# 10XGenomics/scan-rs

Measured on NVIDIA B200. Metric: normalize+PCA cells/s, 1.3Mx33.5k, k=10, higher is better.
Workload: dtype f64

## Files before the change

### profiles/microbench/ring_rate.cu

```cuda
#include <cstdio>
#include <cstdint>
#include <cuda_runtime.h>
#include "../../scan_rs_b200/csrc/tc05.cuh"
using namespace tc05;

template <int NSTG, int MPS, int PW, bool SPIN_PROD>
__global__ void __launch_bounds__(32 * (2 + NSTG * PW), 1) k_ring(int stages, long long *out) {
    extern __shared__ __align__(1024) unsigned char smem[];
    __shared__ unsigned long long full[NSTG], empty[NSTG], done;
    __shared__ uint32_t tslot;
    const uint32_t tid = threadIdx.x, warp = tid >> 5, lane = tid & 31;
    for (uint32_t i = tid; i < 96 * 1024 / 4; i += blockDim.x) reinterpret_cast<uint32_t *>(smem)[i] = 0x01010101u;
    if (tid == 0) {
        for (int i = 0; i < NSTG; i++) { mbar_init(smem_u32(&full[i]), PW); mbar_init(smem_u32(&empty[i]), 1); }
        mbar_init(smem_u32(&done), 1);
        mbar_init_fence();
    }
    if (warp == 0) tmem_alloc_512(smem_u32(&tslot));
    fence_async_smem();
    fence_before_sync();
    __syncthreads();
    fence_after_sync();
    const uint32_t tmem = tslot;
    const uint32_t full0 = smem_u32(full), empty0 = smem_u32(empty);
    if (warp == 1) {
        const uint32_t idesc = instr_desc_i8(128, 144, false, false);
        const uint32_t a16 = smem_u32(smem) >> 4, b16 = a16 + (65536 >> 4);
        const uint64_t da_hi = smem_desc(0, 2048, 128), db_hi = smem_desc(0, 144 / 8 * 128, 128);
        const long long t0 = clock64();
        for (int s = 0; s < stages; s++) {
            const uint32_t ss = s % NSTG;
            mbar_spin(full0 + 8 * ss, (s / NSTG) & 1u);
            fence_after_sync();
            if (elect_one()) {
#pragma unroll
                for (int t = 0; t < MPS; t++) mma_i8(tmem, da_hi | (a16 + ss * 256 + (t & 3) * 64), db_hi | (b16 + (t & 7) * 288), idesc, 1u);
                commit(empty0 + 8 * ss);
            }
            __syncwarp();
        }
        if (elect_one()) commit(smem_u32(&done));
        __syncwarp();
        mbar_wait(smem_u32(&done), 0);
        if (lane == 0 && blockIdx.x == 0) out[0] = clock64() - t0;
    } else if (warp >= 2) {
        const int p = warp - 2, ss = p / PW;
        int fills = 0;
        for (int s = ss; s < stages; s += NSTG, fills++) {
            if (fills > 0) { if (SPIN_PROD) mbar_spin(empty0 + 8 * ss, (fills - 1) & 1u); else mbar_wait(empty0 + 8 * ss, (fills - 1) & 1u); }
            fence_async_smem();
            __syncwarp();
            if (lane == 0) mbar_arrive(full0 + 8 * ss);
        }
    }
    __syncthreads();
    if (warp == 0) tmem_dealloc_512(tmem);
}

template <int NSTG, int MPS, int PW, bool SPIN>
void run(long long *d) {
    const int stages = 4096;
    auto k = k_ring<NSTG, MPS, PW, SPIN>;
    cudaFuncSetAttribute(k, cudaFuncAttributeMaxDynamicSharedMemorySize, 96 * 1024);
    k<<<148, 32 * (2 + NSTG * PW), 96 * 1024>>>(stages, d);
    cudaError_t e = cudaDeviceSynchronize();
    long long h = 0;
    cudaMemcpy(&h, d, 8, cudaMemcpyDeviceToHost);
    printf("stages in ring %2d, MMAs per stage %2d, producer warps per stage %d, producers %s: %6.1f cycles per MMA (floor 72.1)  %s\n", NSTG, MPS, PW,
           SPIN ? "spin    " : "try_wait", (double)h / stages / MPS, cudaGetErrorString(e));
}

int main() {
    long long *d;
    cudaMalloc(&d, 8);
    run<4, 4, 2, false>(d);
    run<4, 4, 2, true>(d);
    run<4, 4, 1, false>(d);
    run<8, 2, 1, false>(d);
    run<8, 4, 1, false>(d);
    run<8, 4, 2, false>(d);
    run<4, 8, 2, false>(d);
    run<2, 8, 4, false>(d);
    run<3, 12, 4, false>(d);
    run<3, 12, 4, true>(d);
    run<2, 16, 4, false>(d);
    return 0;
}
```

### scan_rs_b200/csrc/common.cuh

```cuda
#pragma once
#include <cuda_runtime.h>
#include <cublas_v2.h>
#include <cusolverDn.h>
#include "nccl_shim.h"

#include <cstdarg>
#include <cstdint>
#include <cstdio>
#include <cstring>
#include <memory>
#include <algorithm>
#include <string>
#include <vector>

#include "../../include/scanb200.h"
#include "gather_units.h"

typedef uint32_t u32;
typedef uint64_t u64;

void sb_set_error(const char *fmt, ...);
int sb_fail(int code, const char *fmt, ...);

#define SB_CUDA(expr)                                                                         \
    do {                                                                                      \
        cudaError_t _e = (expr);                                                              \
        if (_e != cudaSuccess)                                                                \
            return sb_fail(_e == cudaErrorMemoryAllocation ? SB_ERR_OOM : SB_ERR_CUDA,        \
                           "CUDA error %s at %s:%d: %s", cudaGetErrorName(_e), __FILE__,      \
                           __LINE__, cudaGetErrorString(_e));                                 \
    } while (0)
#define SB_CUBLAS(expr)                                                                       \
    do {                                                                                      \
        cublasStatus_t _s = (expr);                                                           \
        if (_s != CUBLAS_STATUS_SUCCESS)                                                      \
            return sb_fail(SB_ERR_LINALG, "cuBLAS error %d at %s:%d", (int)_s, __FILE__, __LINE__); \
    } while (0)
#define SB_CUSOLVER(expr)                                                                     \
    do {                                                                                      \
        cusolverStatus_t _s = (expr);                                                         \
        if (_s != CUSOLVER_STATUS_SUCCESS)                                                    \
            return sb_fail(SB_ERR_LINALG, "cuSOLVER error %d at %s:%d", (int)_s, __FILE__, __LINE__); \
    } while (0)
#define SB_NCCL(expr)                                                                         \
    do {                                                                                      \
        ncclResult_t _r = (expr);                                                             \
        if (_r != ncclSuccess)                                                                \
            return sb_fail(SB_ERR_NCCL, "NCCL error %s at %s:%d", ncclGetErrorString(_r),     \
                           __FILE__, __LINE__);                                               \
    } while (0)
#define SB_TRY(expr)                 \
    do {                             \
        int _rc = (expr);            \
        if (_rc != SB_OK) return _rc; \
    } while (0)

cudaStream_t sb_alloc_stream();
cudaMemPool_t sb_alloc_pool();
void sb_set_alloc_stream(cudaStream_t s, cudaMemPool_t pool = nullptr);
bool sb_stream_alive(cudaStream_t s);
void *sb_cache_take(cudaStream_t st, size_t bytes);
bool sb_cache_give(cudaStream_t st, void *p, size_t bytes);
void sb_cache_flush(cudaStream_t st);
void sb_cache_configure(cudaStream_t st, size_t cap_bytes);
#define SB_CACHE_MIN_BYTES ((size_t)1 << 20)
void sb_stream_register(cudaStream_t s, bool alive);

template <typename T>
struct DevBuf {
    T *p = nullptr;
    size_t n = 0;
    cudaStream_t st = nullptr;
    DevBuf() {}
    DevBuf(const DevBuf &) = delete;
    DevBuf &operator=(const DevBuf &) = delete;
    ~DevBuf() { release(); }
    void release() {
        if (p && sb_stream_alive(st)) {
            const size_t bytes = (n ? n : 1) * sizeof(T);
            if (bytes < SB_CACHE_MIN_BYTES || !sb_cache_give(st, p, bytes)) cudaFreeAsync(p, st);
        }
        p = nullptr;
        n = 0;
    }
    int alloc(size_t count) {
        release();
        n = count;
        if (count == 0) count = 1;
        st = sb_alloc_stream();
        if (count * sizeof(T) >= SB_CACHE_MIN_BYTES) {
            p = static_cast<T *>(sb_cache_take(st, count * sizeof(T)));
            if (p) return SB_OK;
        }
        cudaMemPool_t pool = sb_alloc_pool();
        cudaError_t e = pool ? cudaMallocFromPoolAsync((void **)&p, count * sizeof(T), pool, st) : cudaMallocAsync((void **)&p, count * sizeof(T), st);
        if (e == cudaErrorMemoryAllocation) {
            cudaGetLastError();
            sb_cache_flush(st);
            e = pool ? cudaMallocFromPoolAsync((void **)&p, count * sizeof(T), pool, st) : cudaMallocAsync((void **)&p, count * sizeof(T), st);
        }
        if (e != cudaSuccess) {
            p = nullptr;
            n = 0;
            cudaGetLastError();
            return sb_fail(e == cudaErrorMemoryAllocation ? SB_ERR_OOM : SB_ERR_CUDA,
                           "cudaMallocAsync of %zu bytes failed: %s", count * sizeof(T), cudaGetErrorString(e));
        }
        return SB_OK;
    }
    int ensure(size_t count) { return count <= n && p ? SB_OK : alloc(count); }
    void swap(DevBuf &o) {
        T *tp = p; p = o.p; o.p = tp;
        size_t tn = n; n = o.n; o.n = tn;
        cudaStream_t ts = st; st = o.st; o.st = ts;
    }
};

enum Phase { PH_SPMM_T = 0, PH_SPMM_N, PH_MOMENTS, PH_REDUCE, PH_DENSE, PH_COMM, PH_UPLOAD, PH_BUILD, PH_OUTPUT, PH_COUNT };

struct sb_ctx {
    int device = 0;
    int sm_count = 148;
    size_t l2_bytes = 0;
    cudaStream_t stream = nullptr;
    cudaMemPool_t pool = nullptr;
    cudaStream_t copy_stream = nullptr;
    cudaStream_t aux_stream = nullptr;
    cudaEvent_t ev_fork = nullptr, ev_join = nullptr;
    bool overlap = false;
    bool overlap_t = false;
    cublasHandle_t cublas = nullptr;
    cusolverDnHandle_t cusolver = nullptr;
    ncclComm_t comm = nullptr;
    int nranks = 1, rank = 0;
    int dense_cap = 2048;
    double dense_min_density = 0.12;
    bool panel_i8 = false;
    int dense_max_count = 15;
    int panel_mode = 2;
    int pl_debug = 0;
    int pl_variant = 3;
    int plane_items_per_cta = 48;
    int plane_cap = 12288;
    int plane_levels = 6;
    double plane_min_density = 0.01;
    bool gemm_skinny = true;
    bool eig_host = true;
    void *eig_pinned = nullptr;
    size_t eig_pinned_bytes = 0;
    int eig_host_declined = 0;
    int upload_chunks = 8;
    bool upload_sync = true;
    bool gather_defer = true;
    int gather_calibrate = 1;
    double gather_seg_cost = 0.0;
    double gather_flush_cost = 5.0;
    int gather_items_per_cta = 1;
    bool use_gather = true;
    bool direct_projection = false;
    bool verify_projection = false;
    bool eig_jacobi = false;
    bool own_dense = true;
    double last_cond_r = 0.0, last_probe_resid = 0.0;
    int last_fallbacks = 0;
    bool profile_on = false;
    std::vector<std::pair<int, std::pair<cudaEvent_t, cudaEvent_t>>> pending;
    std::vector<cudaEvent_t> event_pool;
    sb_profile prof;
    cudaEvent_t t0 = nullptr, t1 = nullptr;
    DevBuf<char> flush_buf;
    DevBuf<char> scratch;
    DevBuf<double> syrk_parts;
    void *pinned = nullptr;
    std::vector<double> omega_cache;
    u64 omega_seed = ~0ull, omega_rows = 0, omega_cols = 0;
    DevBuf<double> omega_dev;
    u64 omega_dev_seed = ~0ull, omega_dev_rows = 0, omega_dev_cols = 0;
};

#define SB_GENE_BITS 22
#define SB_GENE_MASK 0x3FFFFFu
#define SB_MAX_PANEL_CELLS 1024
#define GA_TBLOCK 16384

#define PL_MAX_LEVELS 6
struct PlUnitT {
    u32 g0, nlev;
    u32 lev[3], nkb[3];
    u32 cta0, nctas;
};
struct PlUnitN {
    u32 g0, nlev;
    u32 mt[PL_MAX_LEVELS];
    u32 cta0, nctas;
};
struct PlItem {
    u32 unit, t0, t1;
};
struct PlaneSet {
    bool active = false;
    u32 L = 0;
    u32 G[PL_MAX_LEVELS] = {0, 0, 0, 0, 0, 0};
    u64 ntiles = 0;
    DevBuf<u32> bits[PL_MAX_LEVELS];
    DevBuf<char> units_t, units_n, items_t, items_n;
    DevBuf<u32> counter;
    mutable DevBuf<signed char> ws_bd, ws_bn;
    mutable DevBuf<double> ws_part, ws_scale2;
    mutable DevBuf<unsigned long long> ws_colmax;
    mutable DevBuf<int> ws_ex;
    u32 n_units_t = 0, n_units_n = 0, n_items_t = 0, n_items_n = 0, t_grid = 0, n_grid = 0;
};

struct GatherLayout {
    bool ready = false;
    u32 rows = 0;
    u32 npanels = 0;
    u64 nnz = 0;
    const uint2 *ent = nullptr;
    DevBuf<uint2> ent_own;
    DevBuf<GUnit> units;
    u32 n_units = 0;
    u32 grid = 0;
    DevBuf<u32> cta_first;
    u32 n_items = 0;
    mutable DevBuf<u32> tickets;
    mutable u32 ticket_base = 0;
    DevBuf<u32> slot_gene;
};

struct sb_mat {
    sb_ctx *ctx = nullptr;
    u32 m = 0;
    u64 n = 0;
    u64 n_global = 0;
    u64 cell_offset = 0;
    u64 nnz = 0;
    DevBuf<u64> cm_ptr;
    DevBuf<uint2> cm;
    u32 pc = 0, np = 0, ur = 1;
    DevBuf<uint2> gm;
    DevBuf<u64> gm_base;
    DevBuf<u64> unit_ptr;
    bool have_full_gm = false;
    u32 gd = 0;
    u32 dense_max_count = 15;
    DevBuf<unsigned char> D;
    DevBuf<u32> hot_idx;
    DevBuf<u32> hot_of_gene;
    PlaneSet pl;
    u64 cold_nnz = 0;
    DevBuf<u64> cold_cm_ptr;
    DevBuf<uint2> cold_cm;
    DevBuf<uint2> cold_gm;
    DevBuf<u64> cold_gm_base;
    GatherLayout gn, gt;
    DevBuf<u32> slot_of_gene;
    std::vector<u64> t_seg_len, t_seg_runs;
    std::vector<GUnit> t_units_host;
    std::vector<u32> t_first_host;
    std::vector<double> t_rate;
    int t_calibrated = 0;
    DevBuf<u32> cell_tot;
    bool have_cell_tot = false;
};
#define SB_DENSE_MAX_COUNT 15u
#define SB_DENSE_LUT 16

struct sb_nmat {
    sb_mat *mat = nullptr;
    sb_ctx *ctx = nullptr;
    int kind = 1;
    int log_base = 0;
    DevBuf<double> col_scale;
    DevBuf<double> l1c, inv_l1c;
    DevBuf<double> lk;
    DevBuf<double> row_scale;
    bool has_row_scale = false;
    bool has_offset = false;
    bool v_ones = true;
    DevBuf<double> u;
    DevBuf<double> v;
};

void prof_begin(sb_ctx *ctx, int phase);
void prof_end(sb_ctx *ctx, int phase);
void prof_collect(sb_ctx *ctx);
static inline void count_launch(sb_ctx *ctx, bool own = true) {
    ctx->prof.kernel_launches++;
    if (own) ctx->prof.own_kernel_launches++;
}
struct ProfScope {
    sb_ctx *c;
    int ph;
    ProfScope(sb_ctx *ctx, int phase) : c(ctx), ph(phase) { prof_begin(c, ph); }
    ~ProfScope() { prof_end(c, ph); }
};

int ctx_scratch(sb_ctx *ctx, size_t bytes, void **out);
int comm_allreduce_f64(sb_ctx *ctx, double *buf, size_t count);
int comm_allreduce_u64(sb_ctx *ctx, u64 *buf, size_t count);
int comm_allreduce_max_i32(sb_ctx *ctx, int *host_val);
int comm_allgather_u64_host(sb_ctx *ctx, u64 mine, std::vector<u64> &all);
int agree_status(sb_ctx *ctx, int rc, const char *what);
double percentile_of(std::vector<double> &v, double q);

#define SB_ENTER(ctx_ptr)                         \
    do {                                          \
        SB_CUDA(cudaSetDevice((ctx_ptr)->device)); \
        sb_set_alloc_stream((ctx_ptr)->stream, (ctx_ptr)->pool); \
    } while (0)

struct TraceScope {
    sb_ctx *c;
    const char *name;
    double t0;
    static bool on();
    static int level();
    static double now();
    TraceScope(sb_ctx *ctx, const char *n) : c(ctx), name(n), t0(0) {
        if (on()) {
            cudaStreamSynchronize(c->stream);
            t0 = now();
        }
    }
    ~TraceScope() {
        if (on()) {
            cudaStreamSynchronize(c->stream);
            fprintf(stderr, "[scanb200] %-28s %8.2f ms\n", name, (now() - t0) * 1e3);
        }
    }
};

struct SyncScope {
    sb_ctx *c;
    const char *name;
    double t0;
    SyncScope(sb_ctx *ctx, const char *n) : c(ctx), name(n), t0(0) {
        cudaStreamSynchronize(c->stream);
        if (TraceScope::on()) t0 = TraceScope::now();
    }
    ~SyncScope() {
        cudaStreamSynchronize(c->stream);
        if (TraceScope::on()) fprintf(stderr, "[scanb200] %-28s %8.2f ms\n", name, (TraceScope::now() - t0) * 1e3);
    }
};

static inline unsigned cdiv(u64 a, u64 b) { return (unsigned)((a + b - 1) / b); }
```

### scan_rs_b200/csrc/planes.cu

```cuda
#include <numeric>

#include "common.cuh"
#include "map.cuh"
#include "tc05.cuh"

using namespace tc05;

#define PL_TILE 128u
#define PL_COLS 20u
#define PL_DIG 7u
#define PL_NCOL 144u
#define PL_FIX 54
#define PL_NONE 0xFFFFFFFFu

#define PT_RANGE 1024u
#define PT_B_BYTES (PT_RANGE * PL_NCOL)
#define PT_KCHUNK_BYTES (PL_NCOL / 8 * 128)
#define PT_WORDS 2u
#define PT_STAGE_BYTES (PL_TILE * 32u * PT_WORDS)
#define PT_NSTAGES 8u
#define PT_SUB 2u
#define PT_NSTG (PT_NSTAGES / PT_SUB)
#define PT_PROD_WARPS PT_NSTAGES
#define PL_EPI_WARPS 4u
#define PL_PROD_WARPS 8u
#define PL_THREADS ((PL_EPI_WARPS + 1 + PL_PROD_WARPS) * 32)

#define PN_GROUP 384u
#define PN_A_BYTES (3u * 4096u)
#define PN_B_BYTES (32u * PL_NCOL)
#define PN_STAGE_BYTES (PN_A_BYTES + PN_B_BYTES)
#define PN_NSTAGES 12u
#define PN_SUB 4u
#define PN_NSTG (PN_NSTAGES / PN_SUB)
#define PN_CELLGRP_BYTES (PL_NCOL / 16 * 128)

struct PlDev {
    u32 *bits[PL_MAX_LEVELS];
    u32 G[PL_MAX_LEVELS];
    u32 L;
    u64 ntiles;
    u64 n;
};

static PlDev make_pldev(const sb_mat *mt) {
    PlDev d;
    memset(&d, 0, sizeof(d));
    d.L = mt->pl.L;
    d.ntiles = mt->pl.ntiles;
    d.n = mt->n;
    for (u32 k = 0; k < mt->pl.L; k++) {
        d.bits[k] = mt->pl.bits[k].p;
        d.G[k] = mt->pl.G[k];
    }
    return d;
}

__global__ void k_pl_level_hist(const u64 *__restrict__ ptr, const uint2 *__restrict__ cm, u64 n, u32 m, u32 L, unsigned long long *__restrict__ hist) {
    u64 warp = ((u64)blockIdx.x * blockDim.x + threadIdx.x) >> 5;
    u64 nwarps = ((u64)gridDim.x * blockDim.x) >> 5;
    int lane = threadIdx.x & 31;
    for (u64 c = warp; c < n; c += nwarps) {
        const u64 s = ptr[c], e = ptr[c + 1];
        for (u64 k = s + lane; k < e; k += 32) {
            const uint2 z = cm[k];
            if (z.y >= 1 && z.y <= L) atomicAdd(&hist[(size_t)(z.y - 1) * m + z.x], 1ull);
        }
    }
}

static void units_round(std::vector<u32> &nctas, const std::vector<double> &cost, u32 total) {
    const size_t U = cost.size();
    nctas.assign(U, 1);
    if (U == 0) return;
    double sum = 0.0;
    for (double c : cost) sum += c;
    if (U >= total || sum <= 0.0) return;
    std::vector<double> ideal(U);
    u32 used = 0;
    for (size_t i = 0; i < U; i++) {
        ideal[i] = cost[i] / sum * total;
        nctas[i] = std::max<u32>(1, (u32)ideal[i]);
        used += nctas[i];
    }
    while (used > total) {
        size_t best = 0;
        double worst = -1e300;
        for (size_t i = 0; i < U; i++)
            if (nctas[i] > 1 && (double)nctas[i] - ideal[i] > worst) { worst = (double)nctas[i] - ideal[i]; best = i; }
        nctas[best]--;
        used--;
    }
    while (used < total) {
        size_t best = 0;
        double worst = -1e300;
        for (size_t i = 0; i < U; i++)
            if (ideal[i] - (double)nctas[i] > worst) { worst = ideal[i] - (double)nctas[i]; best = i; }
        nctas[best]++;
        used++;
    }
}

int planes_select(sb_mat *mt, u64 c0, u64 c1) {
    sb_ctx *ctx = mt->ctx;
    PlaneSet &pl = mt->pl;
    pl.active = false;
    pl.L = 0;
    const u32 m = mt->m;
    const u32 Lmax = (u32)std::min<int>(std::max(ctx->plane_levels, 1), PL_MAX_LEVELS);
    if (m < 128 || mt->n_global == 0 || ctx->plane_cap < 128) return SB_OK;
    SyncScope tr(ctx, "build: plane selection");
    DevBuf<u64> d_hist;
    const size_t hn = (size_t)Lmax * m + 1;
    SB_TRY(d_hist.alloc(hn));
    SB_CUDA(cudaMemsetAsync(d_hist.p, 0, hn * sizeof(u64), ctx->stream));
    if (c1 > c0) {
        ProfScope ps(ctx, PH_REDUCE);
        u64 blocks = std::min<u64>(((c1 - c0) * 32 + 255) / 256, (u64)ctx->sm_count * 16);
        k_pl_level_hist<<<(unsigned)std::max<u64>(1, blocks), 256, 0, ctx->stream>>>(mt->cm_ptr.p + c0, mt->cm.p, c1 - c0, m, Lmax,
                                                                                     (unsigned long long *)d_hist.p);
        count_launch(ctx);
    }
    const u64 sample = c1 - c0;
    SB_CUDA(cudaMemcpyAsync(d_hist.p + (hn - 1), &sample, sizeof(u64), cudaMemcpyHostToDevice, ctx->stream));
    SB_TRY(comm_allreduce_u64(ctx, d_hist.p, hn));
    std::vector<u64> h(hn);
    SB_CUDA(cudaMemcpyAsync(h.data(), d_hist.p, hn * sizeof(u64), cudaMemcpyDeviceToHost, ctx->stream));
    SB_CUDA(cudaStreamSynchronize(ctx->stream));
    const double cells = (double)h[hn - 1];
    if (cells <= 0.0) return SB_OK;
    std::vector<u64> tot(m, 0);
    for (u32 k = 0; k < Lmax; k++)
        for (u32 g = 0; g < m; g++) tot[g] += h[(size_t)k * m + g];
    std::vector<u32> order(m);
    std::iota(order.begin(), order.end(), 0u);
    std::stable_sort(order.begin(), order.end(), [&](u32 a, u32 b) { return tot[a] > tot[b]; });
    const u32 cap = std::min<u32>((u32)ctx->plane_cap, m) & ~127u;
    const double thr = ctx->plane_min_density * cells;
    u32 prev = cap;
    u32 L = 0;
    for (u32 k = 0; k < Lmax; k++) {
        u32 G = 0;
        for (u32 b0 = 0; b0 + 128 <= prev; b0 += 128) {
            double s = 0.0;
            for (u32 r = b0; r < b0 + 128; r++) s += (double)h[(size_t)k * m + order[r]];
            if (s / 128.0 < thr) break;
            G = b0 + 128;
        }
        if (G == 0) break;
        pl.G[k] = G;
        prev = G;
        L = k + 1;
    }
    if (L == 0) return SB_OK;
    pl.L = L;
    pl.ntiles = (mt->n + PL_TILE - 1) / PL_TILE;
    const u32 G1 = pl.G[0];
    std::vector<u32> hot(order.begin(), order.begin() + G1), hot_of(m, PL_NONE);
    for (u32 r = 0; r < G1; r++) hot_of[hot[r]] = r;
    SB_TRY(mt->hot_idx.alloc(G1));
    SB_TRY(mt->hot_of_gene.alloc(m));
    SB_CUDA(cudaMemcpyAsync(mt->hot_idx.p, hot.data(), G1 * sizeof(u32), cudaMemcpyHostToDevice, ctx->stream));
    SB_CUDA(cudaMemcpyAsync(mt->hot_of_gene.p, hot_of.data(), (size_t)m * sizeof(u32), cudaMemcpyHostToDevice, ctx->stream));
    for (u32 k = 0; k < L; k++) {
        const size_t words = std::max<size_t>(1, (size_t)pl.ntiles * (pl.G[k] / 32) * PL_TILE);
        SB_TRY(pl.bits[k].alloc(words));
        SB_CUDA(cudaMemsetAsync(pl.bits[k].p, 0, words * sizeof(u32), ctx->stream));
    }
    std::vector<PlUnitT> ut;
    std::vector<double> cost;
    for (u32 g0 = 0; g0 < G1; g0 += PT_RANGE) {
        std::vector<u32> lv;
        for (u32 k = 0; k < L; k++)
            if (pl.G[k] > g0) lv.push_back(k);
        for (size_t i = 0; i < lv.size(); i += 3) {
            PlUnitT u;
            memset(&u, 0, sizeof(u));
            u.g0 = g0;
            double c = 0.0;
            for (size_t j = i; j < std::min(lv.size(), i + 3); j++) {
                const u32 genes = std::min(pl.G[lv[j]], g0 + PT_RANGE) - g0;
                u.lev[u.nlev] = lv[j];
                u.nkb[u.nlev] = genes / 32;
                u.nlev++;
                c += genes;
            }
            c += (u.nlev > 1 ? 250.0 : 100.0) * u.nlev;
            ut.push_back(u);
            cost.push_back(c);
        }
    }
    {
        double total = 0.0;
        for (double c : cost) total += c * (double)pl.ntiles;
        const double target = std::max(1.0, total / ((double)ctx->sm_count * (double)std::max(1, ctx->plane_items_per_cta)));
        std::vector<u32> uo(ut.size());
        std::iota(uo.begin(), uo.end(), 0u);
        std::stable_sort(uo.begin(), uo.end(), [&](u32 x, u32 y) { return cost[x] > cost[y]; });
        std::vector<PlItem> items;
        for (u32 ui : uo) {
            const u64 per = std::max<u64>(1, (u64)(target / cost[ui] + 0.5));
            for (u64 t0 = 0; t0 < pl.ntiles; t0 += per) {
                PlItem it;
                it.unit = ui;
                it.t0 = (u32)t0;
                it.t1 = (u32)std::min<u64>(pl.ntiles, t0 + per);
                items.push_back(it);
            }
        }
        pl.n_units_t = (u32)ut.size();
        SB_TRY(pl.units_t.alloc(std::max<size_t>(1, ut.size()) * sizeof(PlUnitT)));
        if (!ut.empty()) SB_CUDA(cudaMemcpyAsync(pl.units_t.p, ut.data(), ut.size() * sizeof(PlUnitT), cudaMemcpyHostToDevice, ctx->stream));
        pl.n_items_t = (u32)items.size();
        pl.t_grid = (u32)std::min<size_t>((size_t)ctx->sm_count, std::max<size_t>(1, items.size()));
        SB_TRY(pl.items_t.alloc(std::max<size_t>(1, items.size()) * sizeof(PlItem)));
        if (!items.empty()) SB_CUDA(cudaMemcpyAsync(pl.items_t.p, items.data(), items.size() * sizeof(PlItem), cudaMemcpyHostToDevice, ctx->stream));
        SB_TRY(pl.counter.alloc(4));
        SB_CUDA(cudaStreamSynchronize(ctx->stream));
    }
    std::vector<u32> nc;
    u32 at = 0;
    std::vector<PlUnitN> un;
    cost.clear();
    for (u32 g0 = 0; g0 < G1; g0 += PN_GROUP) {
        PlUnitN u;
        memset(&u, 0, sizeof(u));
        u.g0 = g0;
        double c = 0.0;
        for (u32 k = 0; k < L && pl.G[k] > g0; k++) {
            u.mt[k] = (std::min(pl.G[k], g0 + PN_GROUP) - g0) / 128;
            u.nlev = k + 1;
            c += u.mt[k] + 0.5;
        }
        un.push_back(u);
        cost.push_back(c);
    }
    {
        double total = 0.0;
        for (double c : cost) total += c * (double)pl.ntiles;
        const double target = std::max(1.0, total / ((double)ctx->sm_count * 10.0));
        std::vector<u32> uo(un.size());
        std::iota(uo.begin(), uo.end(), 0u);
        std::stable_sort(uo.begin(), uo.end(), [&](u32 x, u32 y) { return cost[x] > cost[y]; });
        std::vector<PlItem> items;
        for (u32 ui : uo) {
            const u64 per = std::min<u64>(std::max<u64>(1, (u64)(target / cost[ui] + 0.5)), (1u << 24) / PL_TILE);
            for (u64 t0 = 0; t0 < pl.ntiles; t0 += per) {
                PlItem it;
                it.unit = ui;
                it.t0 = (u32)t0;
                it.t1 = (u32)std::min<u64>(pl.ntiles, t0 + per);
                items.push_back(it);
            }
        }
        pl.n_items_n = (u32)items.size();
        pl.n_grid = (u32)std::min<size_t>((size_t)ctx->sm_count, std::max<size_t>(1, items.size()));
        SB_TRY(pl.items_n.alloc(std::max<size_t>(1, items.size()) * sizeof(PlItem)));
        if (!items.empty()) SB_CUDA(cudaMemcpyAsync(pl.items_n.p, items.data(), items.size() * sizeof(PlItem), cudaMemcpyHostToDevice, ctx->stream));
        SB_CUDA(cudaStreamSynchronize(ctx->stream));
    }
    pl.n_units_n = (u32)un.size();
    SB_TRY(pl.units_n.alloc(std::max<size_t>(1, un.size()) * sizeof(PlUnitN)));
    SB_CUDA(cudaMemcpyAsync(pl.units_n.p, un.data(), un.size() * sizeof(PlUnitN), cudaMemcpyHostToDevice, ctx->stream));
    SB_CUDA(cudaStreamSynchronize(ctx->stream));
    pl.active = true;
    mt->gd = G1;
    if (TraceScope::on()) {
        fprintf(stderr, "[scanb200] planes: L=%u G =", L);
        for (u32 k = 0; k < L; k++) fprintf(stderr, " %u", pl.G[k]);
        fprintf(stderr, "  (T units %u / %u CTAs, N units %u / %u CTAs)\n", pl.n_units_t, pl.t_grid, pl.n_units_n, pl.n_grid);
    }
    return SB_OK;
}

__global__ void k_split_planes(const u64 *__restrict__ ptr, const uint2 *__restrict__ cm, u64 n, u64 cbase, const u32 *__restrict__ rank_of_gene,
                               PlDev pl, const u64 *__restrict__ new_ptr, u32 *__restrict__ counts, uint2 *__restrict__ out) {
    u64 warp = ((u64)blockIdx.x * blockDim.x + threadIdx.x) >> 5;
    u64 nwarps = ((u64)gridDim.x * blockDim.x) >> 5;
    int lane = threadIdx.x & 31;
    for (u64 c = warp; c < n; c += nwarps) {
        const u64 s = ptr[c], e = ptr[c + 1];
        const u64 wpos = new_ptr ? new_ptr[c] : 0;
        const u64 cell = cbase + c, tile = cell / PL_TILE;
        const u32 cl = (u32)(cell % PL_TILE);
        u32 total = 0;
        for (u64 k0 = s; k0 < e; k0 += 32) {
            const u64 k = k0 + lane;
            const bool valid = k < e;
            const uint2 z = valid ? cm[k] : make_uint2(0, 0);
            const u32 r = valid ? rank_of_gene[z.x] : PL_NONE;
            const bool dense = valid && r != PL_NONE && z.y >= 1 && z.y <= pl.L && r < pl.G[z.y - 1];
            const bool cold = valid && !dense;
            if (out && dense) {
                const u32 lv = z.y - 1;
                atomicOr(pl.bits[lv] + ((tile * (pl.G[lv] / 32) + (r >> 5)) * PL_TILE + cl), 1u << (r & 31));
            }
            const unsigned mask = __ballot_sync(0xffffffffu, cold);
            if (out && cold) out[wpos + total + __popc(mask & ((1u << lane) - 1u))] = z;
            total += __popc(mask);
        }
        if (counts && lane == 0) counts[c] = total;
    }
}

int planes_split_launch(sb_mat *mt, u64 c0, u64 nc, const u64 *new_ptr, u32 *counts, uint2 *out) {
    sb_ctx *ctx = mt->ctx;
    if (nc == 0) return SB_OK;
    if (c0 % PL_TILE) return sb_fail(SB_ERR_UNSUPPORTED, "planes_split: range start %llu is not a multiple of 128", (unsigned long long)c0);
    u64 blocks = std::min<u64>((nc * 32 + 255) / 256, (u64)ctx->sm_count * 16);
    k_split_planes<<<(unsigned)std::max<u64>(1, blocks), 256, 0, ctx->stream>>>(mt->cm_ptr.p + c0, mt->cm.p, nc, c0, mt->hot_of_gene.p, make_pldev(mt),
                                                                                new_ptr, counts, out);
    count_launch(ctx);
    SB_CUDA(cudaGetLastError());
    return SB_OK;
}

__device__ __forceinline__ double finite_or_zero(double x) { return (x == x && fabs(x) < 1.0e300) ? x : 0.0; }

__device__ __forceinline__ void digits7(long long q, signed char (&d)[PL_DIG]) {
#pragma unroll
    for (u32 s = 0; s < PL_DIG; s++) {
        const long long t = ((q + 128) & 255) - 128;
        d[s] = (signed char)t;
        q = (q - t) >> 8;
    }
}

__device__ __forceinline__ void atomic_max_abs(unsigned long long *slot, double v) {
    atomicMax(slot, (unsigned long long)__double_as_longlong(fabs(v)));
}

__global__ void k_pl_scales(const unsigned long long *__restrict__ colmax_bits, double *__restrict__ scale2, int *__restrict__ ex) {
    const u32 c = threadIdx.x;
    if (c >= PL_COLS) return;
    const double mx = __longlong_as_double((long long)colmax_bits[c]);
    int e = 0;
    if (mx > 0.0) frexp(mx, &e);
    scale2[c] = ldexp(1.0, e - PL_FIX);
    ex[c] = PL_FIX - e;
}

__global__ void k_pl_colmax_t(const double *__restrict__ Y, u32 ldy, const u32 *__restrict__ hot_idx, const double *__restrict__ rs, u32 G1, u32 col0,
                              u32 wt, unsigned long long *__restrict__ colmax_bits) {
    const u32 i = blockIdx.x * blockDim.x + threadIdx.x;
    if (i >= G1 * PL_COLS) return;
    const u32 r = i / PL_COLS, c = i - r * PL_COLS;
    if (c >= wt) return;
    const u32 g = hot_idx[r];
    double v = Y[(size_t)g * ldy + col0 + c];
    if (rs) v *= rs[g];
    atomic_max_abs(&colmax_bits[c], finite_or_zero(v));
}

__global__ void k_pl_digits_t(const double *__restrict__ Y, u32 ldy, const u32 *__restrict__ hot_idx, const double *__restrict__ rs, u32 G1, u32 col0,
                              u32 wt, const int *__restrict__ ex, signed char *__restrict__ Bd, u32 split) {
    const u32 i = blockIdx.x * blockDim.x + threadIdx.x;
    if (i >= G1 * PL_COLS) return;
    const u32 r = i / PL_COLS, c = i - r * PL_COLS;
    const u32 g = hot_idx[r];
    double v = c < wt ? Y[(size_t)g * ldy + col0 + c] : 0.0;
    if (rs) v *= rs[g];
    const long long q = __double2ll_rn(ldexp(finite_or_zero(v), ex[c]));
    signed char d[PL_DIG];
    digits7(q, d);
    const u32 range = r / PT_RANGE, k = r - range * PT_RANGE;
    signed char *base = Bd + (size_t)range * PT_B_BYTES + (size_t)(k >> 4) * PT_KCHUNK_BYTES + (k & 15);
#pragma unroll
    for (u32 s = 0; s < PL_DIG; s++) {
        const u32 n = c * PL_DIG + s + ((split && c >= PL_COLS / 2) ? 2u : 0u);
        base[(size_t)(n >> 3) * 128 + (n & 7) * 16] = d[s];
    }
}

__device__ __forceinline__ double i32_to_f64(u32 r) {
    return __hiloint2double(0x43300000, (int)(r ^ 0x80000000u)) - 4503601774854144.0;
}

__device__ __forceinline__ void read_acc(u32 taddr, double (&val)[PL_COLS]) {
    double lo = 0.0, hi = 0.0;
#pragma unroll
    for (u32 cb = 0; cb < PL_NCOL; cb += 16) {
        u32 r[16];
        tmem_ld16(taddr + cb, r);
        tmem_ld_wait();
#pragma unroll
        for (u32 i = 0; i < 16; i++) {
            const u32 n = cb + i;
            if (n < PL_COLS * PL_DIG) {
                const u32 c = n / PL_DIG, s = n - c * PL_DIG;
                const double d = i32_to_f64(r[i]);
                if (s == 0) lo = d;
                else if (s < 4) lo = fma(d, (double)(1u << (8 * s)), lo);
                else if (s == 4) hi = d;
                else hi = fma(d, (double)(1u << (8 * (s - 4))), hi);
                if (s == PL_DIG - 1) val[c] = fma(hi, 4294967296.0, lo);
            }
        }
    }
}

__device__ __forceinline__ void read_acc_fma(u32 taddr, double lk, double (&res)[PL_COLS]) {
    double lo = 0.0, hi = 0.0;
#pragma unroll
    for (u32 cb = 0; cb < PL_NCOL; cb += 16) {
        u32 r[16];
        tmem_ld16(taddr + cb, r);
        tmem_ld_wait();
#pragma unroll
        for (u32 i = 0; i < 16; i++) {
            const u32 n = cb + i;
            if (n < PL_COLS * PL_DIG) {
                const u32 c = n / PL_DIG, s = n - c * PL_DIG;
                const double d = i32_to_f64(r[i]);
                if (s == 0) lo = d;
                else if (s < 4) lo = fma(d, (double)(1u << (8 * s)), lo);
                else if (s == 4) hi = d;
                else hi = fma(d, (double)(1u << (8 * (s - 4))), hi);
                if (s == PL_DIG - 1) res[c] = fma(lk, fma(hi, 4294967296.0, lo), res[c]);
            }
        }
    }
}

__device__ __forceinline__ void read_acc_fma_half(u32 taddr, double lk, double (&res)[PL_COLS / 2]) {
    u32 ra[16], rb[16], rc[16], rd[16], re[8];
    double lo = 0.0, hi = 0.0;
    auto eat = [&](const u32 *r, u32 n0, u32 cnt) {
#pragma unroll
        for (u32 i = 0; i < cnt; i++) {
            const u32 n = n0 + i;
            if (n < (PL_COLS / 2) * PL_DIG) {
                const u32 c = n / PL_DIG, sdig = n - c * PL_DIG;
                const double d = i32_to_f64(r[i]);
                if (sdig == 0) lo = d;
                else if (sdig < 4) lo = fma(d, (double)(1u << (8 * sdig)), lo);
                else if (sdig == 4) hi = d;
                else hi = fma(d, (double)(1u << (8 * (sdig - 4))), hi);
                if (sdig == PL_DIG - 1) res[c] = fma(lk, fma(hi, 4294967296.0, lo), res[c]);
            }
        }
    };
    tmem_ld16(taddr, ra);
    tmem_ld16(taddr + 16, rb);
    tmem_ld_wait();
    tmem_ld16(taddr + 32, rc);
    tmem_ld16(taddr + 48, rd);
    eat(ra, 0, 16);
    eat(rb, 16, 16);
    tmem_ld_wait();
    tmem_ld8(taddr + 64, re);
    eat(rc, 32, 16);
    eat(rd, 48, 16);
    tmem_ld_wait();
    eat(re, 64, 8);
}

template <int V> struct PtLayout;
template <> struct PtLayout<0> {
    static constexpr u32 WARPS = PL_EPI_WARPS + 1 + PT_PROD_WARPS + 1, EPI = PL_EPI_WARPS;
};
template <> struct PtLayout<1> {
    static constexpr u32 WARPS = 8 + 1 + 1 + PT_PROD_WARPS, EPI = 8;
};
struct PtShared {
    unsigned long long full[PT_NSTG], empty[PT_NSTG], tfull[3], tempty[3], item_full[2], item_empty[2], bload;
    u32 tmem;
    u32 item[2];
    u32 pad;
    double scale2[PL_COLS];
};

template <int V>
__global__ void __launch_bounds__(PtLayout<V>::WARPS * 32, 1)
k_planes_t(PlDev pl, const PlUnitT *__restrict__ units, const PlItem *__restrict__ items, u32 n_items, u32 *__restrict__ counter,
           const signed char *__restrict__ Bd, const double *__restrict__ scale2_g, const double *__restrict__ lk, u32 wt,
           double *__restrict__ part, u32 dbg) {
    extern __shared__ __align__(1024) unsigned char smem[];
    unsigned char *sB = smem;
    unsigned char *sA = sB + PT_B_BYTES;
    PtShared *sh = reinterpret_cast<PtShared *>(sA + PT_NSTAGES * PT_STAGE_BYTES);
    using LY = PtLayout<V>;
    constexpr u32 PT_WARPS = LY::WARPS, PT_THREADS = LY::WARPS * 32, EPI = LY::EPI;
    constexpr u32 W_MMA = EPI, W_SCHED = V ? EPI + 1 : PT_WARPS - 1, W_PROD0 = V ? EPI + 2 : EPI + 1;
    const u32 tid = threadIdx.x, warp = tid >> 5, lane = tid & 31;
    const u32 full0 = smem_u32(sh->full), empty0 = smem_u32(sh->empty), tfull0 = smem_u32(sh->tfull), tempty0 = smem_u32(sh->tempty);
    const u32 ifull0 = smem_u32(sh->item_full), iempty0 = smem_u32(sh->item_empty), bload0 = smem_u32(&sh->bload);
    u32 breloads = 0;

    if (tid == 0) {
        for (u32 i = 0; i < PT_NSTG; i++) {
            mbar_init(full0 + 8 * i, PT_SUB);
            mbar_init(empty0 + 8 * i, 1);
        }
        for (u32 i = 0; i < 3; i++) {
            mbar_init(tfull0 + 8 * i, 1);
            mbar_init(tempty0 + 8 * i, EPI);
        }
        mbar_init(bload0, 1);
        for (u32 i = 0; i < 2; i++) {
            mbar_init(ifull0 + 8 * i, 1);
            mbar_init(iempty0 + 8 * i, PT_WARPS - 1);
        }
        mbar_init_fence();
    }
    if (warp == 0) tmem_alloc_512(smem_u32(&sh->tmem));
    if (tid < PL_COLS) sh->scale2[tid] = scale2_g[tid];
    fence_before_sync();
    __syncthreads();
    fence_after_sync();
    const u32 tmem = sh->tmem;
    const u32 sA_addr = smem_u32(sA), sB_addr = smem_u32(sB);
    const u32 idesc = instr_desc_i8(PL_TILE, PL_NCOL, false, false);
    const uint64_t da_hi = smem_desc(0, PL_TILE * 16, 128), db_hi = smem_desc(0, PT_KCHUNK_BYTES, 128);
    const u64 n_pad = pl.ntiles * PL_TILE;
    const bool scheduler = warp == W_SCHED;

    u32 q = 0;
    u32 job = 0;
    u32 fills = 0;
    u32 cur_unit = 0xFFFFFFFFu;
    u32 g0 = 0, nlev = 0, nkb0 = 0, nkb1 = 0, nkb2 = 0, lev0 = 0, lev1 = 0, lev2 = 0, S = 2;

    for (u32 round = 0;; round++) {
        const u32 rs = round & 1u;
        u32 it;
        if (scheduler) {
            if (round >= 2) mbar_wait(iempty0 + 8 * rs, ((round >> 1) - 1) & 1u);
            it = 0;
            if (lane == 0) {
                it = atomicAdd(counter, 1u);
                sh->item[rs] = it;
            }
            it = __shfl_sync(0xffffffffu, it, 0);
            __syncwarp();
            if (lane == 0) mbar_arrive(ifull0 + 8 * rs);
        } else {
            mbar_wait(ifull0 + 8 * rs, (round >> 1) & 1u);
            it = sh->item[rs];
            __syncwarp();
            if (lane == 0) mbar_arrive(iempty0 + 8 * rs);
        }
        if (it >= n_items) break;
        const PlItem item = items[it];
        if (item.unit != cur_unit) {
            fence_before_sync();
            __syncthreads();
            fence_after_sync();
            const PlUnitT un = units[item.unit];
            cur_unit = item.unit;
            g0 = un.g0;
            nlev = un.nlev;
            nkb0 = un.nkb[0];
            nkb1 = nlev > 1 ? un.nkb[1] : 0;
            nkb2 = nlev > 2 ? un.nkb[2] : 0;
            lev0 = un.lev[0];
            lev1 = nlev > 1 ? un.lev[1] : 0;
            lev2 = nlev > 2 ? un.lev[2] : 0;
            S = (nkb0 + nkb1 + nkb2) / PT_WORDS;
            if (V == 1) {
                if (tid == 0) {
                    mbar_expect_tx(bload0, PT_B_BYTES);
                    const signed char *src = Bd + (size_t)(g0 / PT_RANGE) * PT_B_BYTES;
#pragma unroll 1
                    for (u32 o = 0; o < PT_B_BYTES; o += 16384u) bulk_g2s(sB_addr + o, src + o, 16384u, bload0);
                    mbar_arrive(bload0);
                }
                mbar_wait(bload0, breloads & 1u);
                breloads++;
            } else {
                const uint4 *src = reinterpret_cast<const uint4 *>(Bd + (size_t)(g0 / PT_RANGE) * PT_B_BYTES);
                uint4 *dst = reinterpret_cast<uint4 *>(sB);
                for (u32 i = tid; i < PT_B_BYTES / 16; i += PT_THREADS) dst[i] = src[i];
                fence_async_smem();
                __syncthreads();
            }
        }
        const u64 t0 = item.t0, t1 = item.t1;

        if (V == 1 && warp < EPI) {
            const u32 quarter = warp & 3u, half = warp >> 2;
            const u32 row = quarter * 32 + lane;
            double *pu = part + (size_t)item.unit * n_pad * PL_COLS + half * (PL_COLS / 2);
            for (u64 tile = t0; tile < t1; tile++) {
                const u64 cell = tile * PL_TILE + row;
                double res[PL_COLS / 2];
#pragma unroll
                for (u32 j = 0; j < PL_COLS / 2; j++) res[j] = 0.0;
                double L0 = 0.0, L1 = 0.0, L2 = 0.0;
                if (cell < pl.n) {
                    const double *lc = lk + cell * PL_MAX_LEVELS;
                    L0 = lc[lev0];
                    if (nlev > 1) L1 = lc[lev1];
                    if (nlev > 2) L2 = lc[lev2];
                }
                for (u32 a = 0; a < nlev; a++, job++) {
                    const u32 slot = job % 3u;
                    mbar_wait(tfull0 + 8 * slot, (job / 3u) & 1u);
                    fence_after_sync();
                    if (!(dbg & 2u)) read_acc_fma_half(tmem + ((quarter * 32u) << 16) + slot * PL_NCOL + half * 72u, a == 0 ? L0 : (a == 1 ? L1 : L2), res);
                    fence_before_sync();
                    __syncwarp();
                    if (lane == 0) mbar_arrive(tempty0 + 8 * slot);
                }
                if (!(dbg & 1u)) {
                    double2 *o = reinterpret_cast<double2 *>(pu + cell * PL_COLS);
#pragma unroll
                    for (u32 j = 0; j < PL_COLS / 2; j += 2)
                        o[j >> 1] = make_double2(res[j] * sh->scale2[half * (PL_COLS / 2) + j], res[j + 1] * sh->scale2[half * (PL_COLS / 2) + j + 1]);
                }
            }
        } else if (warp < EPI) {
            const u32 row = warp * 32 + lane;
            double *pu = part + (size_t)item.unit * n_pad * PL_COLS;
            for (u64 tile = t0; tile < t1; tile++) {
                const u64 cell = tile * PL_TILE + row;
                double res[PL_COLS];
#pragma unroll
                for (u32 j = 0; j < PL_COLS; j++) res[j] = 0.0;
                double L0 = 0.0, L1 = 0.0, L2 = 0.0;
                if (cell < pl.n) {
                    const double *lc = lk + cell * PL_MAX_LEVELS;
                    L0 = lc[lev0];
                    if (nlev > 1) L1 = lc[lev1];
                    if (nlev > 2) L2 = lc[lev2];
                }
                for (u32 a = 0; a < nlev; a++, job++) {
                    const u32 slot = job % 3u;
                    mbar_wait(tfull0 + 8 * slot, (job / 3u) & 1u);
                    fence_after_sync();
                    if (!(dbg & 2u)) read_acc_fma(tmem + ((warp * 32u) << 16) + slot * PL_NCOL, a == 0 ? L0 : (a == 1 ? L1 : L2), res);
                    fence_before_sync();
                    __syncwarp();
                    if (lane == 0) mbar_arrive(tempty0 + 8 * slot);
                }
                if (!(dbg & 1u)) {
                    double2 *o = reinterpret_cast<double2 *>(pu + cell * PL_COLS);
#pragma unroll
                    for (u32 j = 0; j < PL_COLS; j += 2) o[j >> 1] = make_double2(res[j] * sh->scale2[j], res[j + 1] * sh->scale2[j + 1]);
                }
            }
        } else if (warp == W_MMA) {
            {
                const u32 a16 = sA_addr >> 4, b16 = sB_addr >> 4;
                const u32 a16x = a16 + ((PL_TILE * 16u >> 4) << 16), b16x = b16 + ((PT_KCHUNK_BYTES >> 4) << 16);
                auto level = [&](u32 nkb) {
                    const u32 slot = job % 3u;
                    if (job >= 3u) {
                        mbar_spin(tempty0 + 8 * slot, (job / 3u - 1u) & 1u);
                        fence_after_sync();
                    }
                    const u32 acc = tmem + slot * PL_NCOL;
                    u32 kb = 0;
                    if (V == 1) {
                        for (; kb < nkb; kb += PT_SUB * PT_WORDS) {
                            const u32 sg = q / PT_SUB, ss = sg & (PT_NSTG - 1);
                            mbar_spin(full0 + 8 * ss, (sg / PT_NSTG) & 1u);
                            fence_after_sync();
                            const u32 alo = a16x + ss * (PT_SUB * PT_STAGE_BYTES >> 4), blo = b16x + kb * (2 * PT_KCHUNK_BYTES >> 4);
                            if (elect_one()) {
#pragma unroll
                                for (u32 t = 0; t < PT_SUB * PT_WORDS; t++)
                                    mma_i8_lo<0x4008u, 0x4008u>(acc, alo + t * (PL_TILE * 32 >> 4), blo + t * (2 * PT_KCHUNK_BYTES >> 4), idesc, kb | t);
                                commit(empty0 + 8 * ss);
                            }
                            __syncwarp();
                            q += PT_SUB;
                        }
                    }
                    for (; kb < nkb; kb += PT_SUB * PT_WORDS) {
                        const u32 sg = q / PT_SUB, ss = sg & (PT_NSTG - 1);
                        mbar_spin(full0 + 8 * ss, (sg / PT_NSTG) & 1u);
                        fence_after_sync();
                        const u32 alo = a16 + ss * (PT_SUB * PT_STAGE_BYTES >> 4), blo = b16 + kb * (2 * PT_KCHUNK_BYTES >> 4);
                        if (elect_one()) {
#pragma unroll
                            for (u32 t = 0; t < PT_SUB * PT_WORDS; t++)
                                mma_i8(acc, da_hi | (alo + t * (PL_TILE * 32 >> 4)), db_hi | (blo + t * (2 * PT_KCHUNK_BYTES >> 4)), idesc, kb | t);
                            commit(empty0 + 8 * ss);
                        }
                        __syncwarp();
                        q += PT_SUB;
                    }
                    if (elect_one()) commit(tfull0 + 8 * slot);
                    __syncwarp();
                    job++;
                };
                for (u64 tile = t0; tile < t1; tile++) {
                    level(nkb0);
                    if (nlev > 1) level(nkb1);
                    if (nlev > 2) level(nkb2);
                }
            }
        } else if (!scheduler) {
            const u32 p = warp - W_PROD0;
            const u32 G0 = pl.G[lev0] >> 5, G1w = pl.G[lev1] >> 5, G2w = pl.G[lev2] >> 5;
            const u32 *bits0 = pl.bits[lev0], *bits1 = pl.bits[lev1], *bits2 = pl.bits[lev2];
            const u32 s0 = nkb0 / PT_WORDS, s1 = nkb1 / PT_WORDS;
            u64 tile = t0;
            u32 i = (p + PT_NSTAGES - (q & (PT_NSTAGES - 1))) & (PT_NSTAGES - 1);
            while (i >= S && tile < t1) {
                i -= S;
                tile++;
            }
            auto load_words = [&](u64 tl, u32 ii, u32 (&w)[4 * PT_WORDS]) {
                const bool in1 = ii >= s0, in2 = ii >= s0 + s1;
                const u32 sb = ii - (in2 ? s0 + s1 : (in1 ? s0 : 0u));
                const u32 Gw = in2 ? G2w : (in1 ? G1w : G0);
                const u32 *bp = in2 ? bits2 : (in1 ? bits1 : bits0);
                const u32 *base = bp + ((size_t)tl * Gw + (g0 >> 5) + sb * PT_WORDS) * PL_TILE + lane;
#pragma unroll
                for (u32 j = 0; j < PT_WORDS; j++)
#pragma unroll
                    for (u32 c4 = 0; c4 < 4; c4++) w[j * 4 + c4] = __ldg(base + (size_t)j * PL_TILE + c4 * 32);
            };
            auto prefetch_tile = [&](u64 tl) {
                if (tl >= t1) return;
                const u32 line = p * (128 / PT_NSTAGES) + lane;
                if (lane < 128 / PT_NSTAGES) {
                    if (line < nkb0 * 4) prefetch_l2(bits0 + ((size_t)tl * G0 + (g0 >> 5)) * PL_TILE + line * 32);
                    if (line < nkb1 * 4) prefetch_l2(bits1 + ((size_t)tl * G1w + (g0 >> 5)) * PL_TILE + line * 32);
                    if (line < nkb2 * 4) prefetch_l2(bits2 + ((size_t)tl * G2w + (g0 >> 5)) * PL_TILE + line * 32);
                }
            };
            u32 cur[4 * PT_WORDS], nxt[4 * PT_WORDS];
            bool live = tile < t1;
            if (live) {
                prefetch_tile(tile + 1);
                prefetch_tile(tile + 2);
                load_words(tile, i, cur);
            }
            const u32 st = sA_addr + p * PT_STAGE_BYTES + lane * 16;
            while (live) {
                u64 ntile = tile;
                u32 ni = i + PT_NSTAGES;
                while (ni >= S && ntile < t1) {
                    ni -= S;
                    ntile++;
                }
                const bool more = ntile < t1;
                if (more) load_words(ntile, ni, nxt);
                if (ntile != tile) prefetch_tile(ntile + 2);
                if (V == 1) {
                    uint4 ex[8];
#pragma unroll
                    for (u32 c4 = 0; c4 < 4; c4++) expand_bits32(cur[c4], ex[2 * c4], ex[2 * c4 + 1]);
                    if (fills > 0) mbar_wait(empty0 + 8 * (p / PT_SUB), (fills - 1) & 1u);
                    if (!(dbg & 4u)) {
#pragma unroll
                        for (u32 c4 = 0; c4 < 4; c4++) {
                            st_shared_v4(st + c4 * 512, ex[2 * c4]);
                            st_shared_v4(st + (PL_TILE * 16) + c4 * 512, ex[2 * c4 + 1]);
                        }
#pragma unroll
                        for (u32 j = 1; j < PT_WORDS; j++)
#pragma unroll
                            for (u32 c4 = 0; c4 < 4; c4++) {
                                uint4 lo, hi;
                                expand_bits32(cur[j * 4 + c4], lo, hi);
                                st_shared_v4(st + (2 * j) * (PL_TILE * 16) + c4 * 512, lo);
                                st_shared_v4(st + (2 * j + 1) * (PL_TILE * 16) + c4 * 512, hi);
                            }
                    }
                } else {
                if (fills > 0) mbar_wait(empty0 + 8 * (p / PT_SUB), (fills - 1) & 1u);
                if (!(dbg & 4u))
#pragma unroll
                    for (u32 j = 0; j < PT_WORDS; j++)
#pragma unroll
                        for (u32 c4 = 0; c4 < 4; c4++) {
                            uint4 lo, hi;
                            expand_bits32(cur[j * 4 + c4], lo, hi);
                            st_shared_v4(st + (2 * j) * (PL_TILE * 16) + c4 * 512, lo);
                            st_shared_v4(st + (2 * j + 1) * (PL_TILE * 16) + c4 * 512, hi);
                        }
                }
                fence_async_smem();
                __syncwarp();
                if (lane == 0) mbar_arrive(full0 + 8 * (p / PT_SUB));
                fills++;
                tile = ntile;
                i = ni;
                live = more;
                if (more) {
#pragma unroll
                    for (u32 c = 0; c < 4 * PT_WORDS; c++) cur[c] = nxt[c];
                }
            }
            q += (u32)(t1 - t0) * S;
        }
    }
    fence_before_sync();
    __syncthreads();
    if (warp == 0) tmem_dealloc_512(tmem);
}

__global__ void k_pl_reduce_t(const double *__restrict__ part, u32 n_units, u64 n, u64 n_pad, u32 col0, u32 wt, double *__restrict__ out, u32 ldo,
                              const double *__restrict__ t1, const double *__restrict__ l1) {
    const u64 total = n * (PL_COLS / 2);
    for (u64 i = (u64)blockIdx.x * blockDim.x + threadIdx.x; i < total; i += (u64)gridDim.x * blockDim.x) {
        const u64 c = i / (PL_COLS / 2);
        const u32 j = (u32)(i - c * (PL_COLS / 2)) * 2;
        if (j >= wt) continue;
        double2 s = make_double2(0.0, 0.0);
        for (u32 u = 0; u < n_units; u++) {
            const double2 v = *reinterpret_cast<const double2 *>(part + ((size_t)u * n_pad + c) * PL_COLS + j);
            s.x += v.x;
            s.y += v.y;
        }
        if (t1) {
            const double2 v = *reinterpret_cast<const double2 *>(t1 + c * PL_COLS + j);
            const double f = l1[c];
            s.x = fma(f, v.x, s.x);
            s.y = fma(f, v.y, s.y);
        }
        double *o = out + c * (size_t)ldo + col0 + j;
        o[0] += s.x;
        if (j + 1 < wt) o[1] += s.y;
    }
}

__global__ void k_pl_colmax_n(const double *__restrict__ X, u32 ldx, u64 n, const double *__restrict__ lk, u32 Ltop, u32 col0, u32 wt,
                              int mode, unsigned long long *__restrict__ colmax_bits) {
    double mx[PL_COLS];
#pragma unroll
    for (u32 j = 0; j < PL_COLS; j++) mx[j] = 0.0;
    for (u64 c = (u64)blockIdx.x * blockDim.x + threadIdx.x; c < n; c += (u64)gridDim.x * blockDim.x) {
        const double l = lk[c * PL_MAX_LEVELS + Ltop - 1];
        if (mode == 1) {
            mx[0] = fmax(mx[0], fabs(l));
            mx[1] = fmax(mx[1], l * l);
        } else {
#pragma unroll
            for (u32 j = 0; j < PL_COLS; j++)
                if (j < wt) mx[j] = fmax(mx[j], fabs(finite_or_zero(l * X[c * (size_t)ldx + col0 + j])));
        }
    }
#pragma unroll
    for (u32 j = 0; j < PL_COLS; j++) {
        double v = mx[j];
        for (int o = 16; o > 0; o >>= 1) v = fmax(v, __shfl_xor_sync(0xffffffffu, v, o));
        if ((threadIdx.x & 31) == 0 && v > 0.0) atomic_max_abs(&colmax_bits[j], v);
    }
}

__global__ void k_pl_digits_n(const double *__restrict__ X, u32 ldx, u64 n, u64 n_pad, const double *__restrict__ lk, u32 L, u32 col0,
                              u32 wt, int mode, const int *__restrict__ ex, signed char *__restrict__ Bn) {
    const u64 i = (u64)blockIdx.x * blockDim.x + threadIdx.x;
    if (i >= n_pad * L) return;
    const u32 lv = (u32)(i / n_pad);
    const u64 c = i - (u64)lv * n_pad;
    u32 pk[PL_NCOL / 4];
#pragma unroll
    for (u32 t = 0; t < PL_NCOL / 4; t++) pk[t] = 0u;
    if (c < n) {
        const double l = lk[c * PL_MAX_LEVELS + lv];
#pragma unroll
        for (u32 j = 0; j < PL_COLS; j++) {
            double v = 0.0;
            if (mode == 1) v = j == 0 ? l : (j == 1 ? l * l : 0.0);
            else if (j < wt) v = finite_or_zero(l * X[c * (size_t)ldx + col0 + j]);
            const long long q = __double2ll_rn(ldexp(v, ex[j]));
            signed char d[PL_DIG];
            digits7(q, d);
#pragma unroll
            for (u32 s = 0; s < PL_DIG; s++) {
                const u32 nn = j * PL_DIG + s;
                pk[nn >> 2] |= (u32)(unsigned char)d[s] << (8 * (nn & 3));
            }
        }
    }
    uint4 *dst = reinterpret_cast<uint4 *>(Bn + ((size_t)lv * (n_pad / 8) + (c >> 3)) * PN_CELLGRP_BYTES + (c & 7) * 16);
#pragma unroll
    for (u32 t = 0; t < PL_NCOL / 16; t++) dst[t * 8] = make_uint4(pk[4 * t], pk[4 * t + 1], pk[4 * t + 2], pk[4 * t + 3]);
}

struct PnShared {
    unsigned long long full[PN_NSTG], empty[PN_NSTG], tfull;
    u32 tmem;
    u32 item[2];
    u32 pad;
    double scale2[PL_COLS];
};

template <int V>
__global__ void __launch_bounds__((PL_EPI_WARPS + 1 + (V ? 12 : 8)) * 32, 1)
k_planes_n(PlDev pl, const PlUnitN *__restrict__ units, const PlItem *__restrict__ items, u32 n_items, u32 *__restrict__ counter,
           const signed char *__restrict__ Bn, u64 n_pad, const double *__restrict__ scale2_g, const u32 *__restrict__ hot_idx, u32 col0, u32 wt,
           double *__restrict__ out, u64 row_stride, u64 col_stride) {
    extern __shared__ __align__(1024) unsigned char smem[];
    unsigned char *sS = smem;
    PnShared *sh = reinterpret_cast<PnShared *>(sS + PN_NSTAGES * PN_STAGE_BYTES);
    const u32 tid = threadIdx.x, warp = tid >> 5, lane = tid & 31;
    const u32 full0 = smem_u32(sh->full), empty0 = smem_u32(sh->empty), tfull0 = smem_u32(&sh->tfull);
    constexpr u32 PW = V ? 12u : 8u;
    if (tid == 0) {
        for (u32 i = 0; i < PN_NSTG; i++) {
            mbar_init(full0 + 8 * i, PN_SUB);
            mbar_init(empty0 + 8 * i, 1);
        }
        mbar_init(tfull0, 1);
        mbar_init_fence();
        sh->item[0] = atomicAdd(counter, 1u);
    }
    if (warp == 0) tmem_alloc_512(smem_u32(&sh->tmem));
    if (tid < PL_COLS) sh->scale2[tid] = scale2_g[tid];
    fence_before_sync();
    __syncthreads();
    fence_after_sync();
    const u32 tmem = sh->tmem;
    const u32 sS_addr = smem_u32(sS);
    const u32 idesc = instr_desc_i8(128, PL_NCOL, true, true);
    const uint64_t da_hi = smem_desc(0, 128, 512);
    const uint64_t db_hi = smem_desc(0, PN_CELLGRP_BYTES, 128);

    u32 sg = 0;
    u32 Q0 = 0;
    for (u32 round = 0;; round++) {
        const u32 it = sh->item[round & 1];
        if (it >= n_items) break;
        if (tid == 0) sh->item[(round + 1) & 1] = atomicAdd(counter, 1u);
        const PlItem item = items[it];
        const PlUnitN un = units[item.unit];
        const u32 nlev = un.nlev, g0w = un.g0 >> 5;
        u32 mt_pack = 0;
        for (u32 k = 0; k < nlev; k++) mt_pack |= un.mt[k] << (4 * k);
        const u64 t_begin = item.t0, t_end = item.t1;

        if (warp < PL_EPI_WARPS) {
            mbar_wait_sleep(tfull0, round & 1u);
            fence_after_sync();
            const u32 row = warp * 32 + lane;
            for (u32 mtile = 0; mtile < (mt_pack & 15u); mtile++) {
                double val[PL_COLS];
                read_acc(tmem + ((warp * 32u) << 16) + mtile * PL_NCOL, val);
                const u32 g = hot_idx[un.g0 + mtile * 128 + row];
                double *o = out + (size_t)g * row_stride;
#pragma unroll
                for (u32 j = 0; j < PL_COLS; j++)
                    if (j < wt && val[j] != 0.0) atomicAdd(o + (size_t)(col0 + j) * col_stride, val[j] * sh->scale2[j]);
            }
        } else if (warp == PL_EPI_WARPS) {
            const u32 s16 = sS_addr >> 4;
            u32 started = 0;
            for (u64 tile = t_begin; tile < t_end; tile++) {
                u32 mtp = mt_pack;
                for (u32 k = 0; k < nlev; k++, mtp >>= 4, sg++) {
                    const u32 slot = sg % PN_NSTG;
                    mbar_spin(full0 + 8 * slot, (sg / PN_NSTG) & 1u);
                    fence_after_sync();
                    const u32 nmt = mtp & 15u;
                    if (V == 1) {
                        if (elect_one()) {
#pragma unroll
                            for (u32 ks = 0; ks < PN_SUB; ks++) {
                                const u32 alo = s16 + (slot * PN_SUB + ks) * (PN_STAGE_BYTES >> 4) + ((128u >> 4) << 16);
                                const u32 blo = s16 + (slot * PN_SUB + ks) * (PN_STAGE_BYTES >> 4) + (PN_A_BYTES >> 4) + ((PN_CELLGRP_BYTES >> 4) << 16);
                                mma_i8_lo<0x4020u, 0x4008u>(tmem, alo, blo, idesc, (started & 1u) | ks);
                                if (nmt > 1) mma_i8_lo<0x4020u, 0x4008u>(tmem + PL_NCOL, alo + 256, blo, idesc, ((started >> 1) & 1u) | ks);
                                if (nmt > 2) mma_i8_lo<0x4020u, 0x4008u>(tmem + 2 * PL_NCOL, alo + 512, blo, idesc, ((started >> 2) & 1u) | ks);
                            }
                            commit(empty0 + 8 * slot);
                        }
                    } else if (elect_one()) {
#pragma unroll
                        for (u32 ks = 0; ks < PN_SUB; ks++) {
                            const u32 alo = s16 + (slot * PN_SUB + ks) * (PN_STAGE_BYTES >> 4);
                            const uint64_t db = db_hi | (alo + (PN_A_BYTES >> 4));
                            mma_i8(tmem, da_hi | alo, db, idesc, (started & 1u) | ks);
                            if (nmt > 1) mma_i8(tmem + PL_NCOL, da_hi | (alo + 256), db, idesc, ((started >> 1) & 1u) | ks);
                            if (nmt > 2) mma_i8(tmem + 2 * PL_NCOL, da_hi | (alo + 512), db, idesc, ((started >> 2) & 1u) | ks);
                        }
                        commit(empty0 + 8 * slot);
                    }
                    __syncwarp();
                    started |= (1u << nmt) - 1u;
                }
            }
            if (elect_one()) commit(tfull0);
            __syncwarp();
        } else {
            const u32 p = warp - (PL_EPI_WARPS + 1);
            const u32 per_tile = PN_SUB * nlev;
            u32 cur[12], nxt[12];
            u64 tile = t_begin;
            u32 r = (p + PW - (Q0 % PW)) % PW;
            u32 Q = Q0 + r;
            while (r >= per_tile && tile < t_end) {
                r -= per_tile;
                tile++;
            }
            auto load_words = [&](u64 tl, u32 ks, u32 k, u32 (&w)[12]) {
                const u32 nw = ((mt_pack >> (4 * k)) & 15u) * 4;
                const u32 *base = pl.bits[k] + ((size_t)tl * (pl.G[k] >> 5) + g0w) * PL_TILE + ks * 32 + lane;
#pragma unroll
                for (u32 j = 0; j < 12; j++) w[j] = (j < nw) ? __ldg(base + (size_t)j * PL_TILE) : 0u;
            };
            auto prefetch_tile = [&](u64 tl) {
                if (tl >= t_end) return;
                for (u32 kk = 0; kk < nlev; kk++) {
                    const u32 alines = ((mt_pack >> (4 * kk)) & 15u) * 16;
                    const u32 line = p * 32 + lane;
                    if (line < alines) prefetch_l2(pl.bits[kk] + ((size_t)tl * (pl.G[kk] >> 5) + g0w) * PL_TILE + line * 32);
                    else if (line - alines < 144) prefetch_l2(Bn + ((size_t)kk * (n_pad / 8) + tl * (PL_TILE / 8)) * PN_CELLGRP_BYTES + (size_t)(line - alines) * 128);
                }
            };
            bool live = tile < t_end;
            u32 ks = r & 3u, k = r >> 2;
            if (live) {
                prefetch_tile(tile + 1);
                prefetch_tile(tile + 2);
                load_words(tile, ks, k, cur);
            }
            while (live) {
                u64 ntile = tile;
                u32 nr = r + PW;
                while (nr >= per_tile) {
                    nr -= per_tile;
                    ntile++;
                }
                const bool more = ntile < t_end;
                const u32 nks = nr & 3u, nk = nr >> 2;
                if (more) load_words(ntile, nks, nk, nxt);
                if (ntile != tile) prefetch_tile(ntile + 2);
                const uint4 *bsrc = reinterpret_cast<const uint4 *>(Bn + ((size_t)k * (n_pad / 8) + (tile * PL_TILE + ks * 32) / 8) * PN_CELLGRP_BYTES);
                uint4 bv[V ? 1 : PN_B_BYTES / 16 / 32];
                if (V == 0) {
#pragma unroll
                    for (u32 t = 0; t < PN_B_BYTES / 16 / 32; t++) bv[V ? 0 : t] = __ldg(bsrc + lane + 32 * t);
                }
                const u32 nw = ((mt_pack >> (4 * k)) & 15u) * 4;
                const u32 sgq = Q / PN_SUB, slot = sgq % PN_NSTG, sub = Q % PN_NSTAGES;
                if (sgq >= PN_NSTG) mbar_wait(empty0 + 8 * slot, (sgq / PN_NSTG - 1) & 1u);
                const u32 st = sS_addr + sub * PN_STAGE_BYTES;
                if (V == 1 && lane == 0) {
                    mbar_expect_tx(full0 + 8 * slot, PN_B_BYTES);
                    bulk_g2s(st + PN_A_BYTES, bsrc, PN_B_BYTES, full0 + 8 * slot);
                }
#pragma unroll
                for (u32 j = 0; j < 12; j++) {
                    if (j < nw) {
                        uint4 lo, hi;
                        expand_bits32(cur[j], lo, hi);
                        const u32 a0 = st + (j >> 2) * 4096 + (2 * (j & 3)) * 512 + lane * 16;
                        st_shared_v4(a0, lo);
                        st_shared_v4(a0 + 512, hi);
                    }
                }
                if (V == 0) {
#pragma unroll
                    for (u32 t = 0; t < PN_B_BYTES / 16 / 32; t++) st_shared_v4(st + PN_A_BYTES + (lane + 32 * t) * 16, bv[V ? 0 : t]);
                }
                fence_async_smem();
                __syncwarp();
                if (lane == 0) mbar_arrive(full0 + 8 * slot);
                Q += PW;
                tile = ntile;
                r = nr;
                ks = nks;
                k = nk;
                live = more;
                if (more) {
#pragma unroll
                    for (u32 j = 0; j < 12; j++) cur[j] = nxt[j];
                }
            }
        }
        Q0 += (u32)(t_end - t_begin) * PN_SUB * nlev;
        fence_before_sync();
        __syncthreads();
        fence_after_sync();
    }
    fence_before_sync();
    __syncthreads();
    if (warp == 0) tmem_dealloc_512(tmem);
}

static int scales_from_colmax(sb_ctx *ctx, DevBuf<unsigned long long> &colmax, DevBuf<double> &scale2, DevBuf<int> &ex) {
    SB_TRY(scale2.ensure(PL_COLS));
    SB_TRY(ex.ensure(PL_COLS));
    k_pl_scales<<<1, 32, 0, ctx->stream>>>(colmax.p, scale2.p, ex.p);
    count_launch(ctx);
    return SB_OK;
}

int gather_run_tile(sb_ctx *ctx, const GatherLayout &L, int mode, const MapDev &mp, u64 n_cells, const double *B, u32 ldb, u32 w, u32 col0, double *out,
                    u32 ldo, long long *cycles);

int planes_t(sb_nmat *a, const double *Y, u32 ldy, u32 w, double *out, u32 ldo, const GatherLayout *gl, const MapDev *mp, long long *cycles) {
    sb_mat *mt = a->mat;
    sb_ctx *ctx = mt->ctx;
    const PlaneSet &pl = mt->pl;
    if (!pl.active || mt->n == 0 || w == 0) return SB_OK;
    const u32 G1 = pl.G[0];
    const u32 nranges = (G1 + PT_RANGE - 1) / PT_RANGE;
    const u64 n_pad = pl.ntiles * PL_TILE;
    DevBuf<unsigned long long> &colmax = pl.ws_colmax;
    DevBuf<signed char> &Bd = pl.ws_bd;
    DevBuf<double> &scale2 = pl.ws_scale2, &part = pl.ws_part;
    DevBuf<int> &ex = pl.ws_ex;
    SB_TRY(colmax.ensure(PL_COLS));
    SB_TRY(Bd.ensure((size_t)nranges * PT_B_BYTES));
    SB_TRY(part.ensure((size_t)(pl.n_units_t + (gl ? 1 : 0)) * n_pad * PL_COLS));
    double *t1 = gl ? part.p + (size_t)pl.n_units_t * n_pad * PL_COLS : nullptr;
    const double *rs = a->has_row_scale ? a->row_scale.p : nullptr;
    const size_t smem = (size_t)PT_B_BYTES + PT_NSTAGES * PT_STAGE_BYTES + sizeof(PtShared);
    const bool v1 = ctx->pl_variant & 1;
    cudaError_t e = v1 ? cudaFuncSetAttribute(k_planes_t<1>, cudaFuncAttributeMaxDynamicSharedMemorySize, (int)smem)
                       : cudaFuncSetAttribute(k_planes_t<0>, cudaFuncAttributeMaxDynamicSharedMemorySize, (int)smem);
    if (e != cudaSuccess) return sb_fail(SB_ERR_CUDA, "planes_t: %zu B of shared memory: %s", smem, cudaGetErrorString(e));
    const u32 items = G1 * PL_COLS;
    const unsigned rblocks = (unsigned)std::max<u64>(1, std::min<u64>((mt->n * (PL_COLS / 2) + 255) / 256, (u64)ctx->sm_count * 16));
    for (u32 col0 = 0; col0 < w; col0 += PL_COLS) {
        const u32 wt = std::min(PL_COLS, w - col0);
        SB_CUDA(cudaMemsetAsync(colmax.p, 0, PL_COLS * sizeof(unsigned long long), ctx->stream));
        if (col0 == 0) SB_CUDA(cudaMemsetAsync(Bd.p, 0, (size_t)nranges * PT_B_BYTES, ctx->stream));
        k_pl_colmax_t<<<cdiv(items, 256), 256, 0, ctx->stream>>>(Y, ldy, mt->hot_idx.p, rs, G1, col0, wt, colmax.p);
        SB_TRY(scales_from_colmax(ctx, colmax, scale2, ex));
        k_pl_digits_t<<<cdiv(items, 256), 256, 0, ctx->stream>>>(Y, ldy, mt->hot_idx.p, rs, G1, col0, wt, ex.p, Bd.p, v1 ? 1u : 0u);
        SB_CUDA(cudaMemsetAsync(pl.counter.p, 0, sizeof(u32), ctx->stream));
        if (gl) {
            SB_CUDA(cudaMemsetAsync(t1, 0, (size_t)mt->n * PL_COLS * sizeof(double), ctx->stream));
            SB_TRY(gather_run_tile(ctx, *gl, 2, *mp, mt->n, Y, ldy, w, col0, t1 - col0, PL_COLS, col0 == 0 ? cycles : nullptr));
        }
        if (v1)
            k_planes_t<1><<<pl.t_grid, PtLayout<1>::WARPS * 32, smem, ctx->stream>>>(make_pldev(mt), (const PlUnitT *)pl.units_t.p,
                                                                                     (const PlItem *)pl.items_t.p, pl.n_items_t, pl.counter.p, Bd.p, scale2.p,
                                                                                     a->lk.p, wt, part.p, (u32)ctx->pl_debug);
        else
            k_planes_t<0><<<pl.t_grid, PtLayout<0>::WARPS * 32, smem, ctx->stream>>>(make_pldev(mt), (const PlUnitT *)pl.units_t.p,
                                                                                     (const PlItem *)pl.items_t.p, pl.n_items_t, pl.counter.p, Bd.p, scale2.p,
                                                                                     a->lk.p, wt, part.p, (u32)ctx->pl_debug);
        k_pl_reduce_t<<<rblocks, 256, 0, ctx->stream>>>(part.p, pl.n_units_t, mt->n, n_pad, col0, wt, out, ldo, t1, gl ? a->l1c.p : nullptr);
        count_launch(ctx); count_launch(ctx); count_launch(ctx); count_launch(ctx);
    }
    SB_CUDA(cudaGetLastError());
    return SB_OK;
}

static int planes_n_impl(sb_nmat *a, const double *X, u32 ldx, u32 w, int mode, double *out, u64 row_stride, u64 col_stride) {
    sb_mat *mt = a->mat;
    sb_ctx *ctx = mt->ctx;
    const PlaneSet &pl = mt->pl;
    if (!pl.active || mt->n == 0 || w == 0) return SB_OK;
    const u64 n_pad = pl.ntiles * PL_TILE;
    DevBuf<unsigned long long> &colmax = pl.ws_colmax;
    DevBuf<signed char> &Bn = pl.ws_bn;
    DevBuf<double> &scale2 = pl.ws_scale2;
    DevBuf<int> &ex = pl.ws_ex;
    SB_TRY(colmax.ensure(PL_COLS));
    SB_TRY(Bn.ensure((size_t)pl.L * (n_pad / 8) * PN_CELLGRP_BYTES));
    const size_t smem = (size_t)PN_NSTAGES * PN_STAGE_BYTES + sizeof(PnShared);
    const bool v1 = ctx->pl_variant & 2;
    cudaError_t e = v1 ? cudaFuncSetAttribute(k_planes_n<1>, cudaFuncAttributeMaxDynamicSharedMemorySize, (int)smem)
                       : cudaFuncSetAttribute(k_planes_n<0>, cudaFuncAttributeMaxDynamicSharedMemorySize, (int)smem);
    if (e != cudaSuccess) return sb_fail(SB_ERR_CUDA, "planes_n: %zu B of shared memory: %s", smem, cudaGetErrorString(e));
    const int cm_blocks = (int)std::max<u64>(1, std::min<u64>((mt->n + 255) / 256, (u64)ctx->sm_count * 4));
    for (u32 col0 = 0; col0 < w; col0 += PL_COLS) {
        const u32 wt = std::min(PL_COLS, w - col0);
        SB_CUDA(cudaMemsetAsync(colmax.p, 0, PL_COLS * sizeof(unsigned long long), ctx->stream));
        k_pl_colmax_n<<<cm_blocks, 256, 0, ctx->stream>>>(X, ldx, mt->n, a->lk.p, pl.L, col0, wt, mode, colmax.p);
        SB_TRY(scales_from_colmax(ctx, colmax, scale2, ex));
        k_pl_digits_n<<<cdiv(n_pad * pl.L, 128), 128, 0, ctx->stream>>>(X, ldx, mt->n, n_pad, a->lk.p, pl.L, col0, wt, mode, ex.p, Bn.p);
        SB_CUDA(cudaMemsetAsync(pl.counter.p, 0, sizeof(u32), ctx->stream));
        if (v1)
            k_planes_n<1><<<pl.n_grid, (PL_EPI_WARPS + 1 + 12) * 32, smem, ctx->stream>>>(make_pldev(mt), (const PlUnitN *)pl.units_n.p,
                                                                                          (const PlItem *)pl.items_n.p, pl.n_items_n, pl.counter.p, Bn.p, n_pad,
                                                                                          scale2.p, mt->hot_idx.p, col0, wt, out, row_stride, col_stride);
        else
            k_planes_n<0><<<pl.n_grid, PL_THREADS, smem, ctx->stream>>>(make_pldev(mt), (const PlUnitN *)pl.units_n.p, (const PlItem *)pl.items_n.p,
                                                                        pl.n_items_n, pl.counter.p, Bn.p, n_pad, scale2.p, mt->hot_idx.p, col0, wt, out,
                                                                        row_stride, col_stride);
        count_launch(ctx); count_launch(ctx); count_launch(ctx);
    }
    SB_CUDA(cudaGetLastError());
    return SB_OK;
}

int planes_n(sb_nmat *a, const double *X, u32 ldx, u32 w, double *P, u32 ldp) { return planes_n_impl(a, X, ldx, w, 0, P, ldp, 1); }

int planes_moments(sb_nmat *a, double *S1, double *S2) {
    if (S2 < S1) return sb_fail(SB_ERR_UNSUPPORTED, "planes_moments: S2 must follow S1");
    return planes_n_impl(a, nullptr, 0, 2, 1, S1, 1, (u64)(S2 - S1));
}
```

### scan_rs_b200/csrc/tc05.cuh

```cuda
#pragma once
#include <cstdint>

namespace tc05 {

__device__ __forceinline__ uint32_t smem_u32(const void *p) { return (uint32_t)__cvta_generic_to_shared(p); }

__device__ __forceinline__ uint64_t smem_desc(uint32_t saddr, uint32_t lbo, uint32_t sbo) {
    uint64_t d = 0;
    d |= (uint64_t)((saddr >> 4) & 0x3FFFu);
    d |= (uint64_t)((lbo >> 4) & 0x3FFFu) << 16;
    d |= (uint64_t)((sbo >> 4) & 0x3FFFu) << 32;
    d |= 1ull << 46;
    return d;
}

__host__ __device__ constexpr uint32_t instr_desc_i8(uint32_t M, uint32_t N, bool a_mn, bool b_mn) {
    return (2u << 4) | (1u << 7) | (1u << 10) | ((a_mn ? 1u : 0u) << 15) | ((b_mn ? 1u : 0u) << 16) | ((N >> 3) << 17) | ((M >> 4) << 24);
}

__device__ __forceinline__ void mma_i8(uint32_t tmem_d, uint64_t da, uint64_t db, uint32_t idesc, uint32_t accumulate) {
    asm volatile(
        "{\n\t.reg .pred p;\n\tsetp.ne.b32 p, %4, 0;\n\t"
        "tcgen05.mma.cta_group::1.kind::i8 [%0], %1, %2, %3, {%5, %5, %5, %5}, p;\n\t}\n" ::"r"(tmem_d),
        "l"(da), "l"(db), "r"(idesc), "r"(accumulate), "r"(0u)
        : "memory");
}

template <uint32_t HI_A, uint32_t HI_B>
__device__ __forceinline__ void mma_i8_lo(uint32_t tmem_d, uint32_t a_lo, uint32_t b_lo, uint32_t idesc, uint32_t accumulate) {
    asm volatile(
        "{\n\t.reg .pred p;\n\t.reg .b64 da, db;\n\tsetp.ne.b32 p, %4, 0;\n\t"
        "mov.b64 da, {%1, %6};\n\tmov.b64 db, {%2, %7};\n\t"
        "tcgen05.mma.cta_group::1.kind::i8 [%0], da, db, %3, {%5, %5, %5, %5}, p;\n\t}\n" ::"r"(tmem_d),
        "r"(a_lo), "r"(b_lo), "r"(idesc), "r"(accumulate), "r"(0u), "n"(HI_A), "n"(HI_B)
        : "memory");
}

__device__ __forceinline__ bool elect_one(uint32_t &leader) {
    uint32_t pred = 0;
    asm volatile(
        "{\n\t.reg .pred px;\n\t"
        "elect.sync %1|px, 0xffffffff;\n\t"
        "selp.u32 %0, 1, 0, px;\n\t}\n"
        : "=r"(pred), "=r"(leader));
    return pred != 0;
}
__device__ __forceinline__ bool elect_one() {
    uint32_t leader;
    return elect_one(leader);
}

__device__ __forceinline__ void commit(uint32_t mbar) {
    asm volatile("tcgen05.commit.cta_group::1.mbarrier::arrive::one.shared::cluster.b64 [%0];" ::"r"(mbar) : "memory");
}

__device__ __forceinline__ void mbar_init(uint32_t mbar, uint32_t count) {
    asm volatile("mbarrier.init.shared::cta.b64 [%0], %1;" ::"r"(mbar), "r"(count) : "memory");
}
__device__ __forceinline__ void mbar_init_fence() { asm volatile("fence.mbarrier_init.release.cluster;" ::: "memory"); }
__device__ __forceinline__ void mbar_arrive(uint32_t mbar) {
    asm volatile("{\n\t.reg .b64 st;\n\tmbarrier.arrive.shared::cta.b64 st, [%0];\n\t}\n" ::"r"(mbar) : "memory");
}
__device__ __forceinline__ void mbar_wait(uint32_t mbar, uint32_t parity) {
    asm volatile(
        "{\n\t.reg .pred p;\n\t"
        "TC05_WAIT_%=:\n\t"
        "mbarrier.try_wait.parity.shared::cta.b64 p, [%0], %1;\n\t"
        "@p bra TC05_DONE_%=;\n\t"
        "bra TC05_WAIT_%=;\n\t"
        "TC05_DONE_%=:\n\t}\n" ::"r"(mbar),
        "r"(parity)
        : "memory");
}

__device__ __forceinline__ void mbar_spin(uint32_t mbar, uint32_t parity) {
    uint32_t done = 0;
    while (!done)
        asm volatile("{\n\t.reg .pred p;\n\tmbarrier.test_wait.parity.shared::cta.b64 p, [%1], %2;\n\tselp.u32 %0, 1, 0, p;\n\t}\n"
                     : "=r"(done)
                     : "r"(mbar), "r"(parity)
                     : "memory");
}

__device__ __forceinline__ void mbar_expect_tx(uint32_t mbar, uint32_t bytes) {
    asm volatile("mbarrier.expect_tx.relaxed.cta.shared::cta.b64 [%0], %1;" ::"r"(mbar), "r"(bytes) : "memory");
}
__device__ __forceinline__ void bulk_g2s(uint32_t dst_saddr, const void *src, uint32_t bytes, uint32_t mbar) {
    asm volatile("cp.async.bulk.shared::cluster.global.mbarrier::complete_tx::bytes [%0], [%1], %2, [%3];" ::"r"(dst_saddr), "l"(src), "r"(bytes),
                 "r"(mbar)
                 : "memory");
}

__device__ __forceinline__ bool mbar_test(uint32_t mbar, uint32_t parity) {
    uint32_t done = 0;
    asm volatile("{\n\t.reg .pred p;\n\tmbarrier.test_wait.parity.shared::cta.b64 p, [%1], %2;\n\tselp.u32 %0, 1, 0, p;\n\t}\n"
                 : "=r"(done)
                 : "r"(mbar), "r"(parity)
                 : "memory");
    return done != 0;
}

__device__ __forceinline__ void mbar_wait_sleep(uint32_t mbar, uint32_t parity) {
    uint32_t done = 0;
    while (!done) {
        asm volatile(
            "{\n\t.reg .pred p;\n\t"
            "mbarrier.try_wait.parity.shared::cta.b64 p, [%1], %2;\n\t"
            "selp.u32 %0, 1, 0, p;\n\t}\n"
            : "=r"(done)
            : "r"(mbar), "r"(parity)
            : "memory");
        if (!done) __nanosleep(500);
    }
}

__device__ __forceinline__ void fence_async_smem() { asm volatile("fence.proxy.async.shared::cta;" ::: "memory"); }
__device__ __forceinline__ void fence_before_sync() { asm volatile("tcgen05.fence::before_thread_sync;" ::: "memory"); }
__device__ __forceinline__ void fence_after_sync() { asm volatile("tcgen05.fence::after_thread_sync;" ::: "memory"); }

__device__ __forceinline__ void tmem_alloc_512(uint32_t slot_saddr) {
    asm volatile("tcgen05.alloc.cta_group::1.sync.aligned.shared::cta.b32 [%0], 512;" ::"r"(slot_saddr) : "memory");
    asm volatile("tcgen05.relinquish_alloc_permit.cta_group::1.sync.aligned;" ::: "memory");
}
__device__ __forceinline__ void tmem_dealloc_512(uint32_t taddr) {
    asm volatile("tcgen05.dealloc.cta_group::1.sync.aligned.b32 %0, 512;" ::"r"(taddr) : "memory");
}

__device__ __forceinline__ void tmem_ld16(uint32_t taddr, uint32_t (&r)[16]) {
    asm volatile(
        "tcgen05.ld.sync.aligned.32x32b.x16.b32 {%0,%1,%2,%3,%4,%5,%6,%7,%8,%9,%10,%11,%12,%13,%14,%15}, [%16];"
        : "=r"(r[0]), "=r"(r[1]), "=r"(r[2]), "=r"(r[3]), "=r"(r[4]), "=r"(r[5]), "=r"(r[6]), "=r"(r[7]), "=r"(r[8]), "=r"(r[9]), "=r"(r[10]),
          "=r"(r[11]), "=r"(r[12]), "=r"(r[13]), "=r"(r[14]), "=r"(r[15])
        : "r"(taddr));
}
__device__ __forceinline__ void tmem_ld8(uint32_t taddr, uint32_t (&r)[8]) {
    asm volatile("tcgen05.ld.sync.aligned.32x32b.x8.b32 {%0,%1,%2,%3,%4,%5,%6,%7}, [%8];"
                 : "=r"(r[0]), "=r"(r[1]), "=r"(r[2]), "=r"(r[3]), "=r"(r[4]), "=r"(r[5]), "=r"(r[6]), "=r"(r[7])
                 : "r"(taddr));
}
__device__ __forceinline__ void tmem_ld_wait() { asm volatile("tcgen05.wait::ld.sync.aligned;" ::: "memory"); }

__device__ __forceinline__ void expand_bits32(uint32_t w, uint4 &lo, uint4 &hi) {
    lo.x = ((w & 0xFu) * 0x00204081u) & 0x01010101u;
    lo.y = (((w >> 4) & 0xFu) * 0x00204081u) & 0x01010101u;
    lo.z = (((w >> 8) & 0xFu) * 0x00204081u) & 0x01010101u;
    lo.w = (((w >> 12) & 0xFu) * 0x00204081u) & 0x01010101u;
    hi.x = (((w >> 16) & 0xFu) * 0x00204081u) & 0x01010101u;
    hi.y = (((w >> 20) & 0xFu) * 0x00204081u) & 0x01010101u;
    hi.z = (((w >> 24) & 0xFu) * 0x00204081u) & 0x01010101u;
    hi.w = ((w >> 28) * 0x00204081u) & 0x01010101u;
}

__device__ __forceinline__ void prefetch_l2(const void *p) { asm volatile("prefetch.global.L2 [%0];" ::"l"(p)); }

__device__ __forceinline__ void st_shared_v4(uint32_t saddr, const uint4 &v) {
    asm volatile("st.shared.v4.u32 [%0], {%1, %2, %3, %4};" ::"r"(saddr), "r"(v.x), "r"(v.y), "r"(v.z), "r"(v.w) : "memory");
}

}
```

Baseline: 17.88 million.

## Run transposed planes kernel as 2-CTA cluster with paired tcgen05 MMAs

Rewrites the transposed bit-plane projection kernel to run as a 2-CTA cluster issuing cta_group::2 M256 int8 MMAs. Each CTA holds half of the digit columns in shared memory (N=160 split into halves), and the work items are now tile pairs. The ring grows to 16 sub-stages with 8 epilogue warps, and the grid is sized from the occupancy of the cluster. The aim is to raise tensor-core throughput per MMA issue and halve the B footprint per CTA, at the cost of cross-CTA barrier traffic and added complexity. It also adds paired-MMA microbenchmarks and changes the default variant.

```diff
diff --git a/profiles/microbench/pair_rate.cu b/profiles/microbench/pair_rate.cu
--- /dev/null
+++ b/profiles/microbench/pair_rate.cu
@@ -0,0 +1,137 @@
+#include <cstdio>
+#include <cstdint>
+#include <cuda_runtime.h>
+#include "../../scan_rs_b200/csrc/tc05.cuh"
+using namespace tc05;
+
+__global__ void __cluster_dims__(2, 1, 1) __launch_bounds__(128, 1) k_pair_rate(uint32_t N, int n_acc, int iters, long long *out) {
+    extern __shared__ __align__(1024) unsigned char smem[];
+    __shared__ unsigned long long bar;
+    __shared__ uint32_t tslot;
+    const uint32_t tid = threadIdx.x, warp = tid >> 5, rank = cluster_rank();
+    for (uint32_t i = tid; i < 32 * 1024 / 4; i += 128) reinterpret_cast<uint32_t *>(smem)[i] = 0x01010101u;
+    if (tid == 0) { mbar_init(smem_u32(&bar), 1); mbar_init_fence(); }
+    if (warp == 0) tmem_alloc_512_pair(smem_u32(&tslot));
+    fence_async_smem();
+    fence_before_sync();
+    cluster_sync();
+    fence_after_sync();
+    const uint32_t tmem = tslot;
+    long long t0 = 0, t1 = 0;
+    if (warp == 1) {
+        if (rank == 0 && elect_one()) {
+            const uint32_t idesc = instr_desc_i8(256, N, false, false);
+            const uint32_t a16 = smem_u32(smem) >> 4, b16 = (smem_u32(smem) + 16384) >> 4;
+            const uint32_t alo = a16 + ((2048u >> 4) << 16), blo = b16 + (((N / 2 / 8 * 128) >> 4) << 16);
+            t0 = clock64();
+            for (int i = 0; i < iters; i++) mma_i8_lo_pair<0x4008u, 0x4008u>(tmem + (i % n_acc) * 160, alo, blo, idesc, 1u);
+            commit_pair(smem_u32(&bar), 3);
+        }
+        __syncwarp();
+        mbar_wait_cluster(smem_u32(&bar), 0);
+        t1 = clock64();
+    }
+    fence_before_sync();
+    cluster_sync();
+    if (tid == 32 && rank == 0 && blockIdx.x == 0) out[0] = t1 - t0;
+    if (warp == 0) tmem_dealloc_512_pair(tmem);
+}
+
+template <int NSUB, int SUB, int PSLOTS>
+__global__ void __cluster_dims__(2, 1, 1) __launch_bounds__(32 * (2 + NSUB / PSLOTS), 1) k_pair_ring(int stages, long long *out) {
+    constexpr int NSTG = NSUB / SUB, PWARPS = NSUB / PSLOTS;
+    extern __shared__ __align__(1024) unsigned char smem[];
+    __shared__ unsigned long long full[NSTG], empty[NSTG], done;
+    __shared__ uint32_t tslot;
+    const uint32_t tid = threadIdx.x, warp = tid >> 5, lane = tid & 31, rank = cluster_rank();
+    for (uint32_t i = tid; i < (NSUB * 8192 + 81920) / 4; i += blockDim.x) reinterpret_cast<uint32_t *>(smem)[i] = 0x01010101u;
+    if (tid == 0) {
+        for (int i = 0; i < NSTG; i++) { mbar_init(smem_u32(&full[i]), 2 * SUB); mbar_init(smem_u32(&empty[i]), 1); }
+        mbar_init(smem_u32(&done), 1);
+        mbar_init_fence();
+    }
+    if (warp == 0) tmem_alloc_512_pair(smem_u32(&tslot));
+    fence_async_smem();
+    fence_before_sync();
+    cluster_sync();
+    fence_after_sync();
+    const uint32_t tmem = tslot;
+    const uint32_t full0 = smem_u32(full), empty0 = smem_u32(empty);
+    long long t0 = 0;
+    if (warp == 1) {
+        if (rank == 0) {
+            const uint32_t idesc = instr_desc_i8(256, 160, false, false);
+            const uint32_t a16 = smem_u32(smem) >> 4, b16 = (smem_u32(smem) + NSUB * 8192) >> 4;
+            const uint32_t alo = a16 + ((2048u >> 4) << 16), blo = b16 + ((1280u >> 4) << 16);
+            t0 = clock64();
+            uint32_t kb = 0;
+            for (int s = 0; s < stages; s++) {
+                const uint32_t ss = s % NSTG;
+                mbar_spin_cluster(full0 + 8 * ss, (s / NSTG) & 1u);
+                fence_after_sync();
+                if (elect_one()) {
+#pragma unroll
+                    for (int t = 0; t < 2 * SUB; t++)
+                        mma_i8_lo_pair<0x4008u, 0x4008u>(tmem, alo + ss * (SUB * 8192 >> 4) + t * (4096 >> 4), blo + ((kb + t) & 31) * (2560 >> 4), idesc, 1u);
+                    commit_pair(empty0 + 8 * ss, 3);
+                }
+                __syncwarp();
+                kb += 2 * SUB;
+            }
+            if (elect_one()) commit_pair(smem_u32(&done), 3);
+            __syncwarp();
+        }
+        mbar_wait_cluster(smem_u32(&done), 0);
+        if (lane == 0 && rank == 0 && blockIdx.x == 0) out[0] = clock64() - t0;
+    } else if (warp >= 2) {
+        const int p = warp - 2;
+        const uint32_t full_leader = peer_addr(full0, 0);
+        for (int g = p; g < stages * SUB; g += PWARPS) {
+            const int slot = g % NSUB, st = slot / SUB, use = g / NSUB;
+            if (use > 0) mbar_wait(empty0 + 8 * st, (use - 1) & 1u);
+            fence_async_smem();
+            __syncwarp();
+            if (lane == 0) mbar_arrive_cluster(full_leader + 8 * st);
+        }
+    }
+    fence_before_sync();
+    cluster_sync();
+    if (warp == 0) tmem_dealloc_512_pair(tmem);
+}
+
+template <int NSUB, int SUB, int PSLOTS>
+void run_ring(long long *d) {
+    const int stages = 4096, smem = NSUB * 8192 + 81920;
+    auto k = k_pair_ring<NSUB, SUB, PSLOTS>;
+    cudaFuncSetAttribute(k, cudaFuncAttributeMaxDynamicSharedMemorySize, smem);
+    for (int grid : {2, 148}) {
+        k<<<grid, 32 * (2 + NSUB / PSLOTS), smem>>>(stages, d);
+        cudaError_t e = cudaDeviceSynchronize();
+        long long h = 0;
+        cudaMemcpy(&h, d, 8, cudaMemcpyDeviceToHost);
+        printf("pair ring: sub-stages %2d, MMAs per stage %2d, sub-slots per producer warp %d, CTAs %3d: %6.1f cycles per M256 MMA  %s\n", NSUB, 2 * SUB,
+               PSLOTS, grid, (double)h / stages / (2 * SUB), cudaGetErrorString(e));
+    }
+}
+
+int main() {
+    long long *d, h;
+    cudaMalloc(&d, 8);
+    cudaFuncSetAttribute(k_pair_rate, cudaFuncAttributeMaxDynamicSharedMemorySize, 32 * 1024);
+    const int iters = 4096;
+    for (uint32_t N : {128u, 160u, 256u})
+        for (int n_acc : {1, 3}) {
+            if (n_acc > 1 && N > 160) continue;
+            for (int grid : {2, 148}) {
+                k_pair_rate<<<grid, 128, 32 * 1024>>>(N, n_acc, iters, d);
+                cudaError_t e = cudaDeviceSynchronize();
+                cudaMemcpy(&h, d, 8, cudaMemcpyDeviceToHost);
+                printf("pair MMA: M256 N=%3u K32 accumulators=%d CTAs=%3d : %7.1f cycles per MMA (%s)\n", N, n_acc, grid, (double)h / iters, cudaGetErrorString(e));
+            }
+        }
+    run_ring<8, 2, 1>(d);
+    run_ring<16, 2, 1>(d);
+    run_ring<16, 2, 2>(d);
+    run_ring<16, 4, 2>(d);
+    return 0;
+}
diff --git a/profiles/microbench/ring_rate.cu b/profiles/microbench/ring_rate.cu
--- a/profiles/microbench/ring_rate.cu
+++ b/profiles/microbench/ring_rate.cu
@@ -34,7 +34,7 @@
             fence_after_sync();
             if (elect_one()) {
 #pragma unroll
-                for (int t = 0; t < MPS; t++) mma_i8(tmem, da_hi | (a16 + ss * 256 + (t & 3) * 64), db_hi | (b16 + (t & 7) * 288), idesc, 1u);
+                for (int t = 0; t < MPS; t++) mma_i8(tmem, da_hi | (a16 + ss * 256 + (t & 3) * 64), db_hi | (b16 + (t & 3) * 288), idesc, 1u);
                 commit(empty0 + 8 * ss);
             }
             __syncwarp();
diff --git a/scan_rs_b200/csrc/common.cuh b/scan_rs_b200/csrc/common.cuh
--- a/scan_rs_b200/csrc/common.cuh
+++ b/scan_rs_b200/csrc/common.cuh
@@ -139,7 +139,7 @@
     int dense_max_count = 15;
     int panel_mode = 2;
     int pl_debug = 0;
-    int pl_variant = 3;
+    int pl_variant = 2;
     int plane_items_per_cta = 48;
     int plane_cap = 12288;
     int plane_levels = 6;
diff --git a/scan_rs_b200/csrc/planes.cu b/scan_rs_b200/csrc/planes.cu
--- a/scan_rs_b200/csrc/planes.cu
+++ b/scan_rs_b200/csrc/planes.cu
@@ -14,14 +14,18 @@
 #define PL_NONE 0xFFFFFFFFu
 
 #define PT_RANGE 1024u
-#define PT_B_BYTES (PT_RANGE * PL_NCOL)
-#define PT_KCHUNK_BYTES (PL_NCOL / 8 * 128)
+#define PT_NCOL 160u
+#define PT_HALF (PT_NCOL / 2)
+#define PT_B_BYTES (PT_RANGE * PT_HALF)
+#define PT_KCHUNK_BYTES (PT_HALF / 8 * 128)
 #define PT_WORDS 2u
 #define PT_STAGE_BYTES (PL_TILE * 32u * PT_WORDS)
-#define PT_NSTAGES 8u
+#define PT_NSTAGES 16u
 #define PT_SUB 2u
 #define PT_NSTG (PT_NSTAGES / PT_SUB)
-#define PT_PROD_WARPS PT_NSTAGES
+#define PT_PROD_WARPS 8u
+#define PT_EPI_WARPS 8u
+#define PT_WARPS (PT_EPI_WARPS + 2 + PT_PROD_WARPS)
 #define PL_EPI_WARPS 4u
 #define PL_PROD_WARPS 8u
 #define PL_THREADS ((PL_EPI_WARPS + 1 + PL_PROD_WARPS) * 32)
@@ -100,6 +104,8 @@
         used++;
     }
 }
+
+static int planes_t_pairs(u32 *pairs);
 
 int planes_select(sb_mat *mt, u64 c0, u64 c1) {
     sb_ctx *ctx = mt->ctx;
@@ -191,20 +197,23 @@
         }
     }
     {
+        u32 pairs = 0;
+        SB_TRY(planes_t_pairs(&pairs));
+        const u64 npairs = (pl.ntiles + 1) / 2;
         double total = 0.0;
-        for (double c : cost) total += c * (double)pl.ntiles;
-        const double target = std::max(1.0, total / ((double)ctx->sm_count * (double)std::max(1, ctx->plane_items_per_cta)));
+        for (double c : cost) total += c * (double)npairs;
+        const double target = std::max(1.0, total / ((double)pairs * (double)std::max(1, ctx->plane_items_per_cta)));
         std::vector<u32> uo(ut.size());
         std::iota(uo.begin(), uo.end(), 0u);
         std::stable_sort(uo.begin(), uo.end(), [&](u32 x, u32 y) { return cost[x] > cost[y]; });
         std::vector<PlItem> items;
         for (u32 ui : uo) {
             const u64 per = std::max<u64>(1, (u64)(target / cost[ui] + 0.5));
-            for (u64 t0 = 0; t0 < pl.ntiles; t0 += per) {
+            for (u64 t0 = 0; t0 < npairs; t0 += per) {
                 PlItem it;
                 it.unit = ui;
                 it.t0 = (u32)t0;
-                it.t1 = (u32)std::min<u64>(pl.ntiles, t0 + per);
+                it.t1 = (u32)std::min<u64>(npairs, t0 + per);
                 items.push_back(it);
             }
         }
@@ -212,7 +221,7 @@
         SB_TRY(pl.units_t.alloc(std::max<size_t>(1, ut.size()) * sizeof(PlUnitT)));
         if (!ut.empty()) SB_CUDA(cudaMemcpyAsync(pl.units_t.p, ut.data(), ut.size() * sizeof(PlUnitT), cudaMemcpyHostToDevice, ctx->stream));
         pl.n_items_t = (u32)items.size();
-        pl.t_grid = (u32)std::min<size_t>((size_t)ctx->sm_count, std::max<size_t>(1, items.size()));
+        pl.t_grid = 2 * (u32)std::min<size_t>((size_t)pairs, std::max<size_t>(1, items.size()));
         SB_TRY(pl.items_t.alloc(std::max<size_t>(1, items.size()) * sizeof(PlItem)));
         if (!items.empty()) SB_CUDA(cudaMemcpyAsync(pl.items_t.p, items.data(), items.size() * sizeof(PlItem), cudaMemcpyHostToDevice, ctx->stream));
         SB_TRY(pl.counter.alloc(4));
@@ -268,7 +277,7 @@
     if (TraceScope::on()) {
         fprintf(stderr, "[scanb200] planes: L=%u G =", L);
         for (u32 k = 0; k < L; k++) fprintf(stderr, " %u", pl.G[k]);
-        fprintf(stderr, "  (T units %u / %u CTAs, N units %u / %u CTAs)\n", pl.n_units_t, pl.t_grid, pl.n_units_n, pl.n_grid);
+        fprintf(stderr, "  (T units %u / %u pairs of CTAs, N units %u / %u CTAs)\n", pl.n_units_t, pl.t_grid / 2, pl.n_units_n, pl.n_grid);
     }
     return SB_OK;
 }
@@ -353,7 +362,7 @@
 }
 
 __global__ void k_pl_digits_t(const double *__restrict__ Y, u32 ldy, const u32 *__restrict__ hot_idx, const double *__restrict__ rs, u32 G1, u32 col0,
-                              u32 wt, const int *__restrict__ ex, signed char *__restrict__ Bd, u32 split) {
+                              u32 wt, const int *__restrict__ ex, signed char *__restrict__ Bd) {
     const u32 i = blockIdx.x * blockDim.x + threadIdx.x;
     if (i >= G1 * PL_COLS) return;
     const u32 r = i / PL_COLS, c = i - r * PL_COLS;
@@ -363,11 +372,11 @@
     const long long q = __double2ll_rn(ldexp(finite_or_zero(v), ex[c]));
     signed char d[PL_DIG];
     digits7(q, d);
-    const u32 range = r / PT_RANGE, k = r - range * PT_RANGE;
-    signed char *base = Bd + (size_t)range * PT_B_BYTES + (size_t)(k >> 4) * PT_KCHUNK_BYTES + (k & 15);
+    const u32 range = r / PT_RANGE, k = r - range * PT_RANGE, half = c / (PL_COLS / 2), ch = c - half * (PL_COLS / 2);
+    signed char *base = Bd + (size_t)(2 * range + half) * PT_B_BYTES + (size_t)(k >> 4) * PT_KCHUNK_BYTES + (k & 15);
 #pragma unroll
     for (u32 s = 0; s < PL_DIG; s++) {
-        const u32 n = c * PL_DIG + s + ((split && c >= PL_COLS / 2) ? 2u : 0u);
+        const u32 n = ch * PL_DIG + s;
         base[(size_t)(n >> 3) * 128 + (n & 7) * 16] = d[s];
     }
 }
@@ -394,29 +403,6 @@
                 else if (s == 4) hi = d;
                 else hi = fma(d, (double)(1u << (8 * (s - 4))), hi);
                 if (s == PL_DIG - 1) val[c] = fma(hi, 4294967296.0, lo);
-            }
-        }
-    }
-}
-
-__device__ __forceinline__ void read_acc_fma(u32 taddr, double lk, double (&res)[PL_COLS]) {
-    double lo = 0.0, hi = 0.0;
-#pragma unroll
-    for (u32 cb = 0; cb < PL_NCOL; cb += 16) {
-        u32 r[16];
-        tmem_ld16(taddr + cb, r);
-        tmem_ld_wait();
-#pragma unroll
-        for (u32 i = 0; i < 16; i++) {
-            const u32 n = cb + i;
-            if (n < PL_COLS * PL_DIG) {
-                const u32 c = n / PL_DIG, s = n - c * PL_DIG;
-                const double d = i32_to_f64(r[i]);
-                if (s == 0) lo = d;
-                else if (s < 4) lo = fma(d, (double)(1u << (8 * s)), lo);
-                else if (s == 4) hi = d;
-                else hi = fma(d, (double)(1u << (8 * (s - 4))), hi);
-                if (s == PL_DIG - 1) res[c] = fma(lk, fma(hi, 4294967296.0, lo), res[c]);
             }
         }
     }
@@ -455,13 +441,6 @@
     eat(re, 64, 8);
 }
 
-template <int V> struct PtLayout;
-template <> struct PtLayout<0> {
-    static constexpr u32 WARPS = PL_EPI_WARPS + 1 + PT_PROD_WARPS + 1, EPI = PL_EPI_WARPS;
-};
-template <> struct PtLayout<1> {
-    static constexpr u32 WARPS = 8 + 1 + 1 + PT_PROD_WARPS, EPI = 8;
-};
 struct PtShared {
     unsigned long long full[PT_NSTG], empty[PT_NSTG], tfull[3], tempty[3], item_full[2], item_empty[2], bload;
     u32 tmem;
@@ -470,54 +449,48 @@
     double scale2[PL_COLS];
 };
 
-template <int V>
-__global__ void __launch_bounds__(PtLayout<V>::WARPS * 32, 1)
+__global__ void __cluster_dims__(2, 1, 1) __launch_bounds__(PT_WARPS * 32, 1)
 k_planes_t(PlDev pl, const PlUnitT *__restrict__ units, const PlItem *__restrict__ items, u32 n_items, u32 *__restrict__ counter,
-           const signed char *__restrict__ Bd, const double *__restrict__ scale2_g, const double *__restrict__ lk, u32 wt,
+           const signed char *__restrict__ Bd, const double *__restrict__ scale2_g, const double *__restrict__ lk, u64 n_part,
            double *__restrict__ part, u32 dbg) {
     extern __shared__ __align__(1024) unsigned char smem[];
     unsigned char *sB = smem;
     unsigned char *sA = sB + PT_B_BYTES;
     PtShared *sh = reinterpret_cast<PtShared *>(sA + PT_NSTAGES * PT_STAGE_BYTES);
-    using LY = PtLayout<V>;
-    constexpr u32 PT_WARPS = LY::WARPS, PT_THREADS = LY::WARPS * 32, EPI = LY::EPI;
-    constexpr u32 W_MMA = EPI, W_SCHED = V ? EPI + 1 : PT_WARPS - 1, W_PROD0 = V ? EPI + 2 : EPI + 1;
-    const u32 tid = threadIdx.x, warp = tid >> 5, lane = tid & 31;
+    constexpr u32 EPI = PT_EPI_WARPS, W_MMA = EPI, W_SCHED = EPI + 1, W_PROD0 = EPI + 2;
+    const u32 tid = threadIdx.x, warp = tid >> 5, lane = tid & 31, rank = cluster_rank();
     const u32 full0 = smem_u32(sh->full), empty0 = smem_u32(sh->empty), tfull0 = smem_u32(sh->tfull), tempty0 = smem_u32(sh->tempty);
     const u32 ifull0 = smem_u32(sh->item_full), iempty0 = smem_u32(sh->item_empty), bload0 = smem_u32(&sh->bload);
     u32 breloads = 0;
 
     if (tid == 0) {
         for (u32 i = 0; i < PT_NSTG; i++) {
-            mbar_init(full0 + 8 * i, PT_SUB);
+            mbar_init(full0 + 8 * i, 2 * PT_SUB);
             mbar_init(empty0 + 8 * i, 1);
         }
         for (u32 i = 0; i < 3; i++) {
             mbar_init(tfull0 + 8 * i, 1);
-            mbar_init(tempty0 + 8 * i, EPI);
+            mbar_init(tempty0 + 8 * i, 2 * EPI);
         }
         mbar_init(bload0, 1);
         for (u32 i = 0; i < 2; i++) {
             mbar_init(ifull0 + 8 * i, 1);
-            mbar_init(iempty0 + 8 * i, PT_WARPS - 1);
+            mbar_init(iempty0 + 8 * i, 2 * PT_WARPS - 1);
         }
         mbar_init_fence();
     }
-    if (warp == 0) tmem_alloc_512(smem_u32(&sh->tmem));
+    if (warp == 0) tmem_alloc_512_pair(smem_u32(&sh->tmem));
     if (tid < PL_COLS) sh->scale2[tid] = scale2_g[tid];
     fence_before_sync();
-    __syncthreads();
+    cluster_sync();
     fence_after_sync();
     const u32 tmem = sh->tmem;
     const u32 sA_addr = smem_u32(sA), sB_addr = smem_u32(sB);
-    const u32 idesc = instr_desc_i8(PL_TILE, PL_NCOL, false, false);
-    const uint64_t da_hi = smem_desc(0, PL_TILE * 16, 128), db_hi = smem_desc(0, PT_KCHUNK_BYTES, 128);
-    const u64 n_pad = pl.ntiles * PL_TILE;
-    const bool scheduler = warp == W_SCHED;
+    const u32 idesc = instr_desc_i8(2 * PL_TILE, PT_NCOL, false, false);
+    const bool scheduler = warp == W_SCHED && rank == 0;
 
     u32 q = 0;
     u32 job = 0;
-    u32 fills = 0;
     u32 cur_unit = 0xFFFFFFFFu;
     u32 g0 = 0, nlev = 0, nkb0 = 0, nkb1 = 0, nkb2 = 0, lev0 = 0, lev1 = 0, lev2 = 0, S = 2;
 
@@ -525,26 +498,28 @@
         const u32 rs = round & 1u;
         u32 it;
         if (scheduler) {
-            if (round >= 2) mbar_wait(iempty0 + 8 * rs, ((round >> 1) - 1) & 1u);
+            if (round >= 2) mbar_wait_cluster(iempty0 + 8 * rs, ((round >> 1) - 1) & 1u);
             it = 0;
             if (lane == 0) {
                 it = atomicAdd(counter, 1u);
                 sh->item[rs] = it;
+                st_cluster_u32(peer_addr(smem_u32(&sh->item[rs]), 1), it);
+                mbar_arrive(ifull0 + 8 * rs);
+                mbar_arrive_cluster(peer_addr(ifull0 + 8 * rs, 1));
             }
             it = __shfl_sync(0xffffffffu, it, 0);
             __syncwarp();
-            if (lane == 0) mbar_arrive(ifull0 + 8 * rs);
         } else {
-            mbar_wait(ifull0 + 8 * rs, (round >> 1) & 1u);
+            mbar_wait_cluster(ifull0 + 8 * rs, (round >> 1) & 1u);
             it = sh->item[rs];
             __syncwarp();
-            if (lane == 0) mbar_arrive(iempty0 + 8 * rs);
+            if (lane == 0) mbar_arrive_cluster(peer_addr(iempty0 + 8 * rs, 0));
         }
         if (it >= n_items) break;
         const PlItem item = items[it];
         if (item.unit != cur_unit) {
             fence_before_sync();
-            __syncthreads();
+            cluster_sync();
             fence_after_sync();
             const PlUnitT un = units[item.unit];
             cur_unit = item.unit;
@@ -557,31 +532,27 @@
             lev1 = nlev > 1 ? un.lev[1] : 0;
             lev2 = nlev > 2 ? un.lev[2] : 0;
             S = (nkb0 + nkb1 + nkb2) / PT_WORDS;
-            if (V == 1) {
-                if (tid == 0) {
-                    mbar_expect_tx(bload0, PT_B_BYTES);
-                    const signed char *src = Bd + (size_t)(g0 / PT_RANGE) * PT_B_BYTES;
+            if (tid == 0) {
+                mbar_expect_tx(bload0, PT_B_BYTES);
+                const signed char *src = Bd + (size_t)(2 * (g0 / PT_RANGE) + rank) * PT_B_BYTES;
 #pragma unroll 1
-                    for (u32 o = 0; o < PT_B_BYTES; o += 16384u) bulk_g2s(sB_addr + o, src + o, 16384u, bload0);
-                    mbar_arrive(bload0);
-                }
-                mbar_wait(bload0, breloads & 1u);
-                breloads++;
-            } else {
-                const uint4 *src = reinterpret_cast<const uint4 *>(Bd + (size_t)(g0 / PT_RANGE) * PT_B_BYTES);
-                uint4 *dst = reinterpret_cast<uint4 *>(sB);
-                for (u32 i = tid; i < PT_B_BYTES / 16; i += PT_THREADS) dst[i] = src[i];
-                fence_async_smem();
-                __syncthreads();
-            }
+                for (u32 o = 0; o < PT_B_BYTES; o += 16384u) bulk_g2s(sB_addr + o, src + o, 16384u, bload0);
+                mbar_arrive(bload0);
+            }
+            mbar_wait(bload0, breloads & 1u);
+            breloads++;
+            fence_before_sync();
+            cluster_sync();
+            fence_after_sync();
         }
         const u64 t0 = item.t0, t1 = item.t1;
 
-        if (V == 1 && warp < EPI) {
+        if (warp < EPI) {
             const u32 quarter = warp & 3u, half = warp >> 2;
             const u32 row = quarter * 32 + lane;
-            double *pu = part + (size_t)item.unit * n_pad * PL_COLS + half * (PL_COLS / 2);
-            for (u64 tile = t0; tile < t1; tile++) {
+            double *pu = part + (size_t)item.unit * n_part * PL_COLS + half * (PL_COLS / 2);
+            for (u64 pair = t0; pair < t1; pair++) {
+                const u64 tile = 2 * pair + rank;
                 const u64 cell = tile * PL_TILE + row;
                 double res[PL_COLS / 2];
 #pragma unroll
@@ -597,175 +568,118 @@
                     const u32 slot = job % 3u;
                     mbar_wait(tfull0 + 8 * slot, (job / 3u) & 1u);
                     fence_after_sync();
-                    if (!(dbg & 2u)) read_acc_fma_half(tmem + ((quarter * 32u) << 16) + slot * PL_NCOL + half * 72u, a == 0 ? L0 : (a == 1 ? L1 : L2), res);
+                    if (!(dbg & 2u)) read_acc_fma_half(tmem + ((quarter * 32u) << 16) + slot * PT_NCOL + half * PT_HALF, a == 0 ? L0 : (a == 1 ? L1 : L2), res);
                     fence_before_sync();
                     __syncwarp();
-                    if (lane == 0) mbar_arrive(tempty0 + 8 * slot);
-                }
-                if (!(dbg & 1u)) {
+                    if (lane == 0) mbar_arrive_remote(peer_addr(tempty0 + 8 * slot, 0));
+                }
+                if (!(dbg & 1u) && tile < pl.ntiles) {
                     double2 *o = reinterpret_cast<double2 *>(pu + cell * PL_COLS);
 #pragma unroll
                     for (u32 j = 0; j < PL_COLS / 2; j += 2)
                         o[j >> 1] = make_double2(res[j] * sh->scale2[half * (PL_COLS / 2) + j], res[j + 1] * sh->scale2[half * (PL_COLS / 2) + j + 1]);
                 }
             }
-        } else if (warp < EPI) {
-            const u32 row = warp * 32 + lane;
-            double *pu = part + (size_t)item.unit * n_pad * PL_COLS;
-            for (u64 tile = t0; tile < t1; tile++) {
-                const u64 cell = tile * PL_TILE + row;
-                double res[PL_COLS];
-#pragma unroll
-                for (u32 j = 0; j < PL_COLS; j++) res[j] = 0.0;
-                double L0 = 0.0, L1 = 0.0, L2 = 0.0;
-                if (cell < pl.n) {
-                    const double *lc = lk + cell * PL_MAX_LEVELS;
-                    L0 = lc[lev0];
-                    if (nlev > 1) L1 = lc[lev1];
-                    if (nlev > 2) L2 = lc[lev2];
-                }
-                for (u32 a = 0; a < nlev; a++, job++) {
-                    const u32 slot = job % 3u;
-                    mbar_wait(tfull0 + 8 * slot, (job / 3u) & 1u);
-                    fence_after_sync();
-                    if (!(dbg & 2u)) read_acc_fma(tmem + ((warp * 32u) << 16) + slot * PL_NCOL, a == 0 ? L0 : (a == 1 ? L1 : L2), res);
-                    fence_before_sync();
-                    __syncwarp();
-                    if (lane == 0) mbar_arrive(tempty0 + 8 * slot);
-                }
-                if (!(dbg & 1u)) {
-                    double2 *o = reinterpret_cast<double2 *>(pu + cell * PL_COLS);
-#pragma unroll
-                    for (u32 j = 0; j < PL_COLS; j += 2) o[j >> 1] = make_double2(res[j] * sh->scale2[j], res[j + 1] * sh->scale2[j + 1]);
-                }
-            }
         } else if (warp == W_MMA) {
-            {
-                const u32 a16 = sA_addr >> 4, b16 = sB_addr >> 4;
-                const u32 a16x = a16 + ((PL_TILE * 16u >> 4) << 16), b16x = b16 + ((PT_KCHUNK_BYTES >> 4) << 16);
+            if (rank == 0) {
+                const u32 a16x = (sA_addr >> 4) + ((PL_TILE * 16u >> 4) << 16), b16x = (sB_addr >> 4) + ((PT_KCHUNK_BYTES >> 4) << 16);
                 auto level = [&](u32 nkb) {
                     const u32 slot = job % 3u;
                     if (job >= 3u) {
                         mbar_spin(tempty0 + 8 * slot, (job / 3u - 1u) & 1u);
                         fence_after_sync();
                     }
-                    const u32 acc = tmem + slot * PL_NCOL;
-                    u32 kb = 0;
-                    if (V == 1) {
-                        for (; kb < nkb; kb += PT_SUB * PT_WORDS) {
-                            const u32 sg = q / PT_SUB, ss = sg & (PT_NSTG - 1);
-                            mbar_spin(full0 + 8 * ss, (sg / PT_NSTG) & 1u);
-                            fence_after_sync();
-                            const u32 alo = a16x + ss * (PT_SUB * PT_STAGE_BYTES >> 4), blo = b16x + kb * (2 * PT_KCHUNK_BYTES >> 4);
-                            if (elect_one()) {
-#pragma unroll
-                                for (u32 t = 0; t < PT_SUB * PT_WORDS; t++)
-                                    mma_i8_lo<0x4008u, 0x4008u>(acc, alo + t * (PL_TILE * 32 >> 4), blo + t * (2 * PT_KCHUNK_BYTES >> 4), idesc, kb | t);
-                                commit(empty0 + 8 * ss);
-                            }
-                            __syncwarp();
-                            q += PT_SUB;
-                        }
-                    }
-                    for (; kb < nkb; kb += PT_SUB * PT_WORDS) {
-                        const u32 sg = q / PT_SUB, ss = sg & (PT_NSTG - 1);
+                    const u32 acc = tmem + slot * PT_NCOL;
+                    for (u32 kb = 0; kb < nkb; kb += PT_SUB * PT_WORDS) {
+                        const u32 sg = q / PT_SUB, ss = sg % PT_NSTG;
                         mbar_spin(full0 + 8 * ss, (sg / PT_NSTG) & 1u);
                         fence_after_sync();
-                        const u32 alo = a16 + ss * (PT_SUB * PT_STAGE_BYTES >> 4), blo = b16 + kb * (2 * PT_KCHUNK_BYTES >> 4);
+                        const u32 alo = a16x + ss * (PT_SUB * PT_STAGE_BYTES >> 4), blo = b16x + kb * (2 * PT_KCHUNK_BYTES >> 4);
                         if (elect_one()) {
 #pragma unroll
                             for (u32 t = 0; t < PT_SUB * PT_WORDS; t++)
-                                mma_i8(acc, da_hi | (alo + t * (PL_TILE * 32 >> 4)), db_hi | (blo + t * (2 * PT_KCHUNK_BYTES >> 4)), idesc, kb | t);
-                            commit(empty0 + 8 * ss);
+                                mma_i8_lo_pair<0x4008u, 0x4008u>(acc, alo + t * (PL_TILE * 32 >> 4), blo + t * (2 * PT_KCHUNK_BYTES >> 4), idesc, kb | t);
+                            commit_pair(empty0 + 8 * ss, 3);
                         }
                         __syncwarp();
                         q += PT_SUB;
                     }
-                    if (elect_one()) commit(tfull0 + 8 * slot);
+                    if (elect_one()) commit_pair(tfull0 + 8 * slot, 3);
                     __syncwarp();
                     job++;
                 };
-                for (u64 tile = t0; tile < t1; tile++) {
+                for (u64 pair = t0; pair < t1; pair++) {
                     level(nkb0);
                     if (nlev > 1) level(nkb1);
                     if (nlev > 2) level(nkb2);
                 }
             }
-        } else if (!scheduler) {
+        } else if (warp >= W_PROD0) {
             const u32 p = warp - W_PROD0;
             const u32 G0 = pl.G[lev0] >> 5, G1w = pl.G[lev1] >> 5, G2w = pl.G[lev2] >> 5;
             const u32 *bits0 = pl.bits[lev0], *bits1 = pl.bits[lev1], *bits2 = pl.bits[lev2];
             const u32 s0 = nkb0 / PT_WORDS, s1 = nkb1 / PT_WORDS;
-            u64 tile = t0;
-            u32 i = (p + PT_NSTAGES - (q & (PT_NSTAGES - 1))) & (PT_NSTAGES - 1);
-            while (i >= S && tile < t1) {
+            u64 pair = t0;
+            u32 g = q + ((p + PT_PROD_WARPS - (q % PT_PROD_WARPS)) % PT_PROD_WARPS);
+            u32 i = g - q;
+            while (i >= S && pair < t1) {
                 i -= S;
-                tile++;
-            }
-            auto load_words = [&](u64 tl, u32 ii, u32 (&w)[4 * PT_WORDS]) {
+                pair++;
+            }
+            auto load_words = [&](u64 pr, u32 ii, u32 (&w)[4 * PT_WORDS]) {
+                const u64 tl = 2 * pr + rank;
                 const bool in1 = ii >= s0, in2 = ii >= s0 + s1;
                 const u32 sb = ii - (in2 ? s0 + s1 : (in1 ? s0 : 0u));
                 const u32 Gw = in2 ? G2w : (in1 ? G1w : G0);
                 const u32 *bp = in2 ? bits2 : (in1 ? bits1 : bits0);
                 const u32 *base = bp + ((size_t)tl * Gw + (g0 >> 5) + sb * PT_WORDS) * PL_TILE + lane;
+                const bool real = tl < pl.ntiles;
 #pragma unroll
                 for (u32 j = 0; j < PT_WORDS; j++)
 #pragma unroll
-                    for (u32 c4 = 0; c4 < 4; c4++) w[j * 4 + c4] = __ldg(base + (size_t)j * PL_TILE + c4 * 32);
+                    for (u32 c4 = 0; c4 < 4; c4++) w[j * 4 + c4] = real ? __ldg(base + (size_t)j * PL_TILE + c4 * 32) : 0u;
             };
-            auto prefetch_tile = [&](u64 tl) {
-                if (tl >= t1) return;
-                const u32 line = p * (128 / PT_NSTAGES) + lane;
-                if (lane < 128 / PT_NSTAGES) {
+            auto prefetch_tile = [&](u64 pr) {
+                const u64 tl = 2 * pr + rank;
+                if (pr >= t1 || tl >= pl.ntiles) return;
+                const u32 line = p * (128 / PT_PROD_WARPS) + lane;
+                if (lane < 128 / PT_PROD_WARPS) {
                     if (line < nkb0 * 4) prefetch_l2(bits0 + ((size_t)tl * G0 + (g0 >> 5)) * PL_TILE + line * 32);
                     if (line < nkb1 * 4) prefetch_l2(bits1 + ((size_t)tl * G1w + (g0 >> 5)) * PL_TILE + line * 32);
                     if (line < nkb2 * 4) prefetch_l2(bits2 + ((size_t)tl * G2w + (g0 >> 5)) * PL_TILE + line * 32);
                 }
             };
             u32 cur[4 * PT_WORDS], nxt[4 * PT_WORDS];
-            bool live = tile < t1;
+            bool live = pair < t1;
             if (live) {
-                prefetch_tile(tile + 1);
-                prefetch_tile(tile + 2);
-                load_words(tile, i, cur);
-            }
-            const u32 st = sA_addr + p * PT_STAGE_BYTES + lane * 16;
+                prefetch_tile(pair + 1);
+                prefetch_tile(pair + 2);
+                load_words(pair, i, cur);
+            }
             while (live) {
-                u64 ntile = tile;
-                u32 ni = i + PT_NSTAGES;
-                while (ni >= S && ntile < t1) {
+                u64 npair = pair;
+                u32 ni = i + PT_PROD_WARPS;
+                while (ni >= S && npair < t1) {
                     ni -= S;
-                    ntile++;
-                }
-                const bool more = ntile < t1;
-                if (more) load_words(ntile, ni, nxt);
-                if (ntile != tile) prefetch_tile(ntile + 2);
-                if (V == 1) {
-                    uint4 ex[8];
-#pragma unroll
-                    for (u32 c4 = 0; c4 < 4; c4++) expand_bits32(cur[c4], ex[2 * c4], ex[2 * c4 + 1]);
-                    if (fills > 0) mbar_wait(empty0 + 8 * (p / PT_SUB), (fills - 1) & 1u);
-                    if (!(dbg & 4u)) {
-#pragma unroll
-                        for (u32 c4 = 0; c4 < 4; c4++) {
-                            st_shared_v4(st + c4 * 512, ex[2 * c4]);
-                            st_shared_v4(st + (PL_TILE * 16) + c4 * 512, ex[2 * c4 + 1]);
-                        }
-#pragma unroll
-                        for (u32 j = 1; j < PT_WORDS; j++)
-#pragma unroll
-                            for (u32 c4 = 0; c4 < 4; c4++) {
-                                uint4 lo, hi;
-                                expand_bits32(cur[j * 4 + c4], lo, hi);
-                                st_shared_v4(st + (2 * j) * (PL_TILE * 16) + c4 * 512, lo);
-                                st_shared_v4(st + (2 * j + 1) * (PL_TILE * 16) + c4 * 512, hi);
-                            }
+                    npair++;
+                }
+                const bool more = npair < t1;
+                if (more) load_words(npair, ni, nxt);
+                if (npair != pair) prefetch_tile(npair + 2);
+                const u32 sub = g % PT_NSTAGES, use = g / PT_NSTAGES, stg = sub / PT_SUB;
+                const u32 st = sA_addr + sub * PT_STAGE_BYTES + lane * 16;
+                uint4 ex[8];
+#pragma unroll
+                for (u32 c4 = 0; c4 < 4; c4++) expand_bits32(cur[c4], ex[2 * c4], ex[2 * c4 + 1]);
+                if (use > 0) mbar_wait(empty0 + 8 * stg, (use - 1) & 1u);
+                if (!(dbg & 4u)) {
+#pragma unroll
+                    for (u32 c4 = 0; c4 < 4; c4++) {
+                        st_shared_v4(st + c4 * 512, ex[2 * c4]);
+                        st_shared_v4(st + (PL_TILE * 16) + c4 * 512, ex[2 * c4 + 1]);
                     }
-                } else {
-                if (fills > 0) mbar_wait(empty0 + 8 * (p / PT_SUB), (fills - 1) & 1u);
-                if (!(dbg & 4u))
-#pragma unroll
-                    for (u32 j = 0; j < PT_WORDS; j++)
+#pragma unroll
+                    for (u32 j = 1; j < PT_WORDS; j++)
 #pragma unroll
                         for (u32 c4 = 0; c4 < 4; c4++) {
                             uint4 lo, hi;
@@ -776,9 +690,9 @@
                 }
                 fence_async_smem();
                 __syncwarp();
-                if (lane == 0) mbar_arrive(full0 + 8 * (p / PT_SUB));
-                fills++;
-                tile = ntile;
+                if (lane == 0) mbar_arrive_cluster(peer_addr(full0 + 8 * stg, 0));
+                g += PT_PROD_WARPS;
+                pair = npair;
                 i = ni;
                 live = more;
                 if (more) {
@@ -790,8 +704,25 @@
         }
     }
     fence_before_sync();
-    __syncthreads();
-    if (warp == 0) tmem_dealloc_512(tmem);
+    cluster_sync();
+    if (warp == 0) tmem_dealloc_512_pair(tmem);
+}
+
+static constexpr size_t PT_SMEM = (size_t)PT_B_BYTES + PT_NSTAGES * PT_STAGE_BYTES + sizeof(PtShared);
+
+static int planes_t_pairs(u32 *pairs) {
+    cudaError_t e = cudaFuncSetAttribute(k_planes_t, cudaFuncAttributeMaxDynamicSharedMemorySize, (int)PT_SMEM);
+    if (e != cudaSuccess) return sb_fail(SB_ERR_CUDA, "planes_t: %zu B of shared memory: %s", PT_SMEM, cudaGetErrorString(e));
+    cudaLaunchConfig_t cfg;
+    memset(&cfg, 0, sizeof(cfg));
+    cfg.gridDim = dim3(2, 1, 1);
+    cfg.blockDim = dim3(PT_WARPS * 32, 1, 1);
+    cfg.dynamicSmemBytes = PT_SMEM;
+    int n = 0;
+    e = cudaOccupancyMaxActiveClusters(&n, k_planes_t, &cfg);
+    if (e != cudaSuccess || n < 1) return sb_fail(SB_ERR_CUDA, "planes_t: no resident pair of CTAs: %s", cudaGetErrorString(e));
+    *pairs = (u32)n;
+    return SB_OK;
 }
 
 __global__ void k_pl_reduce_t(const double *__restrict__ part, u32 n_units, u64 n, u64 n_pad, u32 col0, u32 wt, double *__restrict__ out, u32 ldo,
@@ -1093,44 +1024,34 @@
     if (!pl.active || mt->n == 0 || w == 0) return SB_OK;
     const u32 G1 = pl.G[0];
     const u32 nranges = (G1 + PT_RANGE - 1) / PT_RANGE;
-    const u64 n_pad = pl.ntiles * PL_TILE;
+    const u64 n_part = (pl.ntiles + 1) / 2 * (2 * PL_TILE);
     DevBuf<unsigned long long> &colmax = pl.ws_colmax;
     DevBuf<signed char> &Bd = pl.ws_bd;
     DevBuf<double> &scale2 = pl.ws_scale2, &part = pl.ws_part;
     DevBuf<int> &ex = pl.ws_ex;
     SB_TRY(colmax.ensure(PL_COLS));
-    SB_TRY(Bd.ensure((size_t)nranges * PT_B_BYTES));
-    SB_TRY(part.ensure((size_t)(pl.n_units_t + (gl ? 1 : 0)) * n_pad * PL_COLS));
-    double *t1 = gl ? part.p + (size_t)pl.n_units_t * n_pad * PL_COLS : nullptr;
+    SB_TRY(Bd.ensure((size_t)nranges * 2 * PT_B_BYTES));
+    SB_TRY(part.ensure((size_t)(pl.n_units_t + (gl ? 1 : 0)) * n_part * PL_COLS));
+    double *t1 = gl ? part.p + (size_t)pl.n_units_t * n_part * PL_COLS : nullptr;
     const double *rs = a->has_row_scale ? a->row_scale.p : nullptr;
-    const size_t smem = (size_t)PT_B_BYTES + PT_NSTAGES * PT_STAGE_BYTES + sizeof(PtShared);
-    const bool v1 = ctx->pl_variant & 1;
-    cudaError_t e = v1 ? cudaFuncSetAttribute(k_planes_t<1>, cudaFuncAttributeMaxDynamicSharedMemorySize, (int)smem)
-                       : cudaFuncSetAttribute(k_planes_t<0>, cudaFuncAttributeMaxDynamicSharedMemorySize, (int)smem);
-    if (e != cudaSuccess) return sb_fail(SB_ERR_CUDA, "planes_t: %zu B of shared memory: %s", smem, cudaGetErrorString(e));
     const u32 items = G1 * PL_COLS;
     const unsigned rblocks = (unsigned)std::max<u64>(1, std::min<u64>((mt->n * (PL_COLS / 2) + 255) / 256, (u64)ctx->sm_count * 16));
     for (u32 col0 = 0; col0 < w; col0 += PL_COLS) {
         const u32 wt = std::min(PL_COLS, w - col0);
         SB_CUDA(cudaMemsetAsync(colmax.p, 0, PL_COLS * sizeof(unsigned long long), ctx->stream));
-        if (col0 == 0) SB_CUDA(cudaMemsetAsync(Bd.p, 0, (size_t)nranges * PT_B_BYTES, ctx->stream));
+        if (col0 == 0) SB_CUDA(cudaMemsetAsync(Bd.p, 0, (size_t)nranges * 2 * PT_B_BYTES, ctx->stream));
         k_pl_colmax_t<<<cdiv(items, 256), 256, 0, ctx->stream>>>(Y, ldy, mt->hot_idx.p, rs, G1, col0, wt, colmax.p);
         SB_TRY(scales_from_colmax(ctx, colmax, scale2, ex));
-        k_pl_digits_t<<<cdiv(items, 256), 256, 0, ctx->stream>>>(Y, ldy, mt->hot_idx.p, rs, G1, col0, wt, ex.p, Bd.p, v1 ? 1u : 0u);
+        k_pl_digits_t<<<cdiv(items, 256), 256, 0, ctx->stream>>>(Y, ldy, mt->hot_idx.p, rs, G1, col0, wt, ex.p, Bd.p);
         SB_CUDA(cudaMemsetAsync(pl.counter.p, 0, sizeof(u32), ctx->stream));
         if (gl) {
             SB_CUDA(cudaMemsetAsync(t1, 0, (size_t)mt->n * PL_COLS * sizeof(double), ctx->stream));
             SB_TRY(gather_run_tile(ctx, *gl, 2, *mp, mt->n, Y, ldy, w, col0, t1 - col0, PL_COLS, col0 == 0 ? cycles : nullptr));
         }
-        if (v1)
-            k_planes_t<1><<<pl.t_grid, PtLayout<1>::WARPS * 32, smem, ctx->stream>>>(make_pldev(mt), (const PlUnitT *)pl.units_t.p,
-                                                                                     (const PlItem *)pl.items_t.p, pl.n_items_t, pl.counter.p, Bd.p, scale2.p,
-                                                                                     a->lk.p, wt, part.p, (u32)ctx->pl_debug);
-        else
-            k_planes_t<0><<<pl.t_grid, PtLayout<0>::WARPS * 32, smem, ctx->stream>>>(make_pldev(mt), (const PlUnitT *)pl.units_t.p,
-                                                                                     (const PlItem *)pl.items_t.p, pl.n_items_t, pl.counter.p, Bd.p, scale2.p,
-                                                                                     a->lk.p, wt, part.p, (u32)ctx->pl_debug);
-        k_pl_reduce_t<<<rblocks, 256, 0, ctx->stream>>>(part.p, pl.n_units_t, mt->n, n_pad, col0, wt, out, ldo, t1, gl ? a->l1c.p : nullptr);
+        k_planes_t<<<pl.t_grid, PT_WARPS * 32, PT_SMEM, ctx->stream>>>(make_pldev(mt), (const PlUnitT *)pl.units_t.p, (const PlItem *)pl.items_t.p,
+                                                                       pl.n_items_t, pl.counter.p, Bd.p, scale2.p, a->lk.p, n_part, part.p,
+                                                                       (u32)ctx->pl_debug);
+        k_pl_reduce_t<<<rblocks, 256, 0, ctx->stream>>>(part.p, pl.n_units_t, mt->n, n_part, col0, wt, out, ldo, t1, gl ? a->l1c.p : nullptr);
         count_launch(ctx); count_launch(ctx); count_launch(ctx); count_launch(ctx);
     }
     SB_CUDA(cudaGetLastError());
diff --git a/scan_rs_b200/csrc/tc05.cuh b/scan_rs_b200/csrc/tc05.cuh
--- a/scan_rs_b200/csrc/tc05.cuh
+++ b/scan_rs_b200/csrc/tc05.cuh
@@ -34,6 +34,66 @@
         "tcgen05.mma.cta_group::1.kind::i8 [%0], da, db, %3, {%5, %5, %5, %5}, p;\n\t}\n" ::"r"(tmem_d),
         "r"(a_lo), "r"(b_lo), "r"(idesc), "r"(accumulate), "r"(0u), "n"(HI_A), "n"(HI_B)
         : "memory");
+}
+
+__device__ __forceinline__ uint32_t cluster_rank() {
+    uint32_t r;
+    asm volatile("mov.u32 %0, %%cluster_ctarank;" : "=r"(r));
+    return r;
+}
+__device__ __forceinline__ void cluster_sync() {
+    asm volatile("barrier.cluster.arrive.release.aligned;\n\tbarrier.cluster.wait.acquire.aligned;" ::: "memory");
+}
+__device__ __forceinline__ uint32_t peer_addr(uint32_t saddr, uint32_t rank) {
+    uint32_t r;
+    asm volatile("mapa.shared::cluster.u32 %0, %1, %2;" : "=r"(r) : "r"(saddr), "r"(rank));
+    return r;
+}
+__device__ __forceinline__ void mbar_arrive_cluster(uint32_t caddr) {
+    asm volatile("mbarrier.arrive.release.cluster.shared::cluster.b64 _, [%0];" ::"r"(caddr) : "memory");
+}
+__device__ __forceinline__ void mbar_arrive_remote(uint32_t caddr) {
+    asm volatile("mbarrier.arrive.release.cta.shared::cluster.b64 _, [%0];" ::"r"(caddr) : "memory");
+}
+__device__ __forceinline__ void st_cluster_u32(uint32_t caddr, uint32_t v) { asm volatile("st.shared::cluster.u32 [%0], %1;" ::"r"(caddr), "r"(v) : "memory"); }
+__device__ __forceinline__ void mbar_wait_cluster(uint32_t mbar, uint32_t parity) {
+    asm volatile(
+        "{\n\t.reg .pred p;\n\t"
+        "TC05_CWAIT_%=:\n\t"
+        "mbarrier.try_wait.parity.acquire.cluster.shared::cta.b64 p, [%0], %1;\n\t"
+        "@p bra TC05_CDONE_%=;\n\t"
+        "bra TC05_CWAIT_%=;\n\t"
+        "TC05_CDONE_%=:\n\t}\n" ::"r"(mbar),
+        "r"(parity)
+        : "memory");
+}
+__device__ __forceinline__ void mbar_spin_cluster(uint32_t mbar, uint32_t parity) {
+    uint32_t done = 0;
+    while (!done)
+        asm volatile("{\n\t.reg .pred p;\n\tmbarrier.test_wait.parity.acquire.cluster.shared::cta.b64 p, [%1], %2;\n\tselp.u32 %0, 1, 0, p;\n\t}\n"
+                     : "=r"(done)
+                     : "r"(mbar), "r"(parity)
+                     : "memory");
+}
+template <uint32_t HI_A, uint32_t HI_B>
+__device__ __forceinline__ void mma_i8_lo_pair(uint32_t tmem_d, uint32_t a_lo, uint32_t b_lo, uint32_t idesc, uint32_t accumulate) {
+    asm volatile(
+        "{\n\t.reg .pred p;\n\t.reg .b64 da, db;\n\tsetp.ne.b32 p, %4, 0;\n\t"
+        "mov.b64 da, {%1, %5};\n\tmov.b64 db, {%2, %6};\n\t"
+        "tcgen05.mma.cta_group::2.kind::i8 [%0], da, db, %3, p;\n\t}\n" ::"r"(tmem_d),
+        "r"(a_lo), "r"(b_lo), "r"(idesc), "r"(accumulate), "n"(HI_A), "n"(HI_B)
+        : "memory");
+}
+__device__ __forceinline__ void commit_pair(uint32_t mbar, uint16_t cta_mask) {
+    asm volatile("tcgen05.commit.cta_group::2.mbarrier::arrive::one.shared::cluster.multicast::cluster.b64 [%0], %1;" ::"r"(mbar), "h"(cta_mask)
+                 : "memory");
+}
+__device__ __forceinline__ void tmem_alloc_512_pair(uint32_t slot_saddr) {
+    asm volatile("tcgen05.alloc.cta_group::2.sync.aligned.shared::cta.b32 [%0], 512;" ::"r"(slot_saddr) : "memory");
+    asm volatile("tcgen05.relinquish_alloc_permit.cta_group::2.sync.aligned;" ::: "memory");
+}
+__device__ __forceinline__ void tmem_dealloc_512_pair(uint32_t taddr) {
+    asm volatile("tcgen05.dealloc.cta_group::2.sync.aligned.b32 %0, 512;" ::"r"(taddr) : "memory");
 }
 
 __device__ __forceinline__ bool elect_one(uint32_t &leader) {
```

New measurement: 17.16 million (median of 6 runs). 4.0% lower.
